# gc00/simgrid

Measured on AMD Instinct MI355X. Metric: LMM solve throughput (vars/s), higher is better.
Workload: dtype f64

## Files before the change

### include/lmm/lmm_hip.h

```cpp
#ifndef LMM_HIP_H
#define LMM_HIP_H

#include <stdint.h>

#ifdef __cplusplus
extern "C" {
#endif

#define LMMHIP_OK 0
#define LMMHIP_E_NODEVICE (-1)
#define LMMHIP_E_HIP (-2)
#define LMMHIP_E_ARG (-3)
#define LMMHIP_E_STATE (-4)
#define LMMHIP_E_NOCONVERGE (-5)

#define LMMHIP_KIND_MAXMIN 0
#define LMMHIP_KIND_FAIR_BOTTLENECK 1

typedef struct lmmhip_ctx lmmhip_ctx;

typedef struct lmmhip_stats {
  int64_t rounds;
  int64_t n_var, n_cnst, nnz;
  double device_ms;
  double kernel_ms[8];
  int64_t kernel_launches[8];
} lmmhip_stats;

int lmmhip_ctx_create(int device, lmmhip_ctx** out);
int lmmhip_ctx_destroy(lmmhip_ctx* ctx);

int lmmhip_upload(lmmhip_ctx* ctx, int64_t n_var, int64_t n_cnst, int64_t nnz, const int64_t* var_ptr,
                  const int32_t* cnst_idx, const double* weight, const double* penalty, const double* var_bound,
                  const double* cnst_bound, const uint8_t* cnst_flags);

int lmmhip_upload2(lmmhip_ctx* ctx, int64_t n_var, int64_t n_cnst, int64_t nnz, const int64_t* var_ptr,
                   const int32_t* cnst_idx, const double* weight, const double* penalty, const double* var_bound,
                   const double* cnst_bound, const uint8_t* cnst_flags, const int64_t* csc_order);

int lmmhip_update_vars(lmmhip_ctx* ctx, const double* penalty, const double* var_bound);
int lmmhip_update_cnsts(lmmhip_ctx* ctx, const double* cnst_bound);

int lmmhip_res_apply(lmmhip_ctx* ctx, int64_t n_elem_total, int64_t n_var_total, int64_t n_cnst_total, int64_t ne,
                     const int64_t* e_id, const int32_t* e_cnst, const double* e_weight, const uint8_t* e_flags,
                     int64_t nv, const int32_t* v_id, const int64_t* v_ebase, const int32_t* v_nelem,
                     const double* v_penalty, const double* v_bound, int64_t nc, const int32_t* c_id,
                     const double* c_bound, const uint8_t* c_flags);
int lmmhip_res_flatten(lmmhip_ctx* ctx, int64_t n_list, const int32_t* cnst_list, double precision, int64_t* counts3);
int lmmhip_res_flatten_fair(lmmhip_ctx* ctx, int64_t n_list, const int32_t* cnst_list, int64_t* counts3);
int lmmhip_res_values(lmmhip_ctx* ctx, int64_t n, double* values, uint8_t* reset);
int lmmhip_res_values_pinned(lmmhip_ctx* ctx, int64_t n, const double** values, const uint8_t** reset);
#define LMMHIP_VAL_KEEP 0x7FF4C0FFEE5107E5ull
int lmmhip_res_values_sliced(lmmhip_ctx* ctx, int64_t n, int nslices, const double** values);
int lmmhip_res_values_wait(lmmhip_ctx* ctx, int slice);
int lmmhip_res_refreshes(lmmhip_ctx* ctx, int64_t* n);
int lmmhip_res_cross_refreshes(lmmhip_ctx* ctx, int64_t* n);
int lmmhip_flat_download(lmmhip_ctx* ctx, int64_t* counts3, uint32_t* var_ptr, int32_t* csr_c, double* csr_w,
                         uint32_t* cnst_ptr, int32_t* csc_v, double* csc_w, double* penalty, double* var_bound,
                         double* cnst_bound, uint8_t* cnst_flags);

int lmmhip_set_batch(lmmhip_ctx* ctx, int64_t nsys, const int64_t* var_off, const int64_t* cnst_off);

int lmmhip_solve(lmmhip_ctx* ctx, int kind, double precision);

int lmmhip_get_values(lmmhip_ctx* ctx, double* values_out);
int lmmhip_get_var_rounds(lmmhip_ctx* ctx, int32_t* rounds_out);
int lmmhip_get_saturated(lmmhip_ctx* ctx, uint8_t* saturated_out);
int lmmhip_get_usage(lmmhip_ctx* ctx, double* usage_out);
int lmmhip_usage_device_ptr(lmmhip_ctx* ctx, const double** dptr);
typedef struct lmmhip_cert {
  double max_excess;
  int64_t n_infeasible, n_unbottlenecked;
  int64_t n_judged_cnst, n_judged_var, n_at_bound;
} lmmhip_cert;
#define LMMHIP_WIT_AT_BOUND (-1)
#define LMMHIP_WIT_NONE (-2)
#define LMMHIP_WIT_NOT_JUDGED (-3)
int lmmhip_certificate(lmmhip_ctx* ctx, double precision, lmmhip_cert* out, int32_t* witness);
int lmmhip_get_touched_vars(lmmhip_ctx* ctx, int32_t* ids, int64_t cap, int64_t* n);
int lmmhip_get_touched_cnsts(lmmhip_ctx* ctx, int32_t* ids, int64_t cap, int64_t* n);
int lmmhip_components(lmmhip_ctx* ctx, int32_t* var_label, int32_t* cnst_label, int64_t* ncomp);
int lmmhip_values_device_ptr(lmmhip_ctx* ctx, const double** dptr);

int lmmhip_get_stats(lmmhip_ctx* ctx, lmmhip_stats* out);
int lmmhip_set_profiling(lmmhip_ctx* ctx, int on);
int lmmhip_launch_profile(lmmhip_ctx* ctx, int* slot, int* round, float* ms, int cap);
int lmmhip_round_profile(lmmhip_ctx* ctx, int64_t* alive_vars, int64_t* alive_elems, int cap);
int lmmhip_vote_profile(lmmhip_ctx* ctx, int64_t* reeval_vars, int64_t* reeval_elems, int cap);
int lmmhip_vote_diag_profile(lmmhip_ctx* ctx, int64_t* out8, int cap);

int lmmhip_ctx_set_stream(lmmhip_ctx* ctx, void* hip_stream);
int lmmhip_ctx_use_own_stream(lmmhip_ctx* ctx);

#define LMMHIP_ENGINE_PERSISTENT 0
#define LMMHIP_ENGINE_ROUNDS 1
#define LMMHIP_ENGINE_AUTO 2
#define LMMHIP_ENGINE_FRONTIER 3
int lmmhip_ctx_set_engine(lmmhip_ctx* ctx, int engine);
int lmmhip_engine_fallbacks(lmmhip_ctx* ctx, int64_t* n);
#define LMMHIP_RAN_PERSISTENT 0
#define LMMHIP_RAN_ROUNDS 1
#define LMMHIP_RAN_FRONTIER 2
#define LMMHIP_RAN_BATCH 3
#define LMMHIP_RAN_FB_ROUNDS 4
#define LMMHIP_RAN_FB_BATCH 5
int lmmhip_last_engine(lmmhip_ctx* ctx, int* engine);
int lmmhip_anatomy(lmmhip_ctx* ctx, unsigned long long* out, int64_t cap, int64_t* n, int32_t* rounds4);
int lmmhip_persist_profile(lmmhip_ctx* ctx, int on, int64_t* t, int64_t cap, int64_t* n);
int lmmhip_persist_profile_blocks(lmmhip_ctx* ctx, int64_t* t, int64_t cap, int64_t* nbar, int64_t* nblk);

int lmmhip_fb_shard_owner(lmmhip_ctx* ctx, int64_t n_own, const int32_t* own_cnst, const int64_t* optr,
                          const int32_t* ovar, const double* oweight, const int32_t* cpos, int64_t n_mu,
                          int64_t n_rem);
int lmmhip_fb_shard_begin(lmmhip_ctx* ctx, double precision, int32_t* xnb, double* xmu, int64_t mu_off,
                          double* xrem);
int lmmhip_fb_shard_step(lmmhip_ctx* ctx, int phase);
int lmmhip_fb_shard_pack_mu(lmmhip_ctx* ctx, int32_t* pos, double* mu, int32_t* count);
int lmmhip_fb_shard_poll(lmmhip_ctx* ctx, int* done, int64_t* rounds);
int lmmhip_fb_work(lmmhip_ctx* ctx, int64_t* out3);

#define LMMHIP_MODEL_CPU 0
#define LMMHIP_MODEL_CM02 1
#define LMMHIP_MODEL_L07 2
#define LMMHIP_EV_FINISHED 1
#define LMMHIP_EV_LATENCY_PAID 2
int lmmhip_actions_upload(lmmhip_ctx* ctx, int64_t n, const int32_t* var_index, const double* remains,
                          const double* max_duration, const double* latency, const double* penalty,
                          const double* sharing_penalty, const uint8_t* flags);
int lmmhip_next_event_full(lmmhip_ctx* ctx, int with_latency, double* out);
int lmmhip_update_actions_full(lmmhip_ctx* ctx, int model, double delta, double maxmin_precision,
                               double surf_precision, int64_t* n_events);
int lmmhip_actions_download(lmmhip_ctx* ctx, double* remains, double* max_duration, double* latency, double* penalty,
                            uint8_t* events);

#define LMMHIP_HEAP_UNSET 0
#define LMMHIP_HEAP_LATENCY 1
#define LMMHIP_HEAP_MAX_DURATION 2
#define LMMHIP_HEAP_NORMAL 3
#define LMMHIP_ACT_NOT_STARTED 4
int lmmhip_actions_lazy_upload(lmmhip_ctx* ctx, const double* last_update, const double* last_value,
                               const double* start_time, const double* date, const uint8_t* heap_type);
int lmmhip_actions_lazy_update(lmmhip_ctx* ctx, int model, double now, double maxmin_precision, double surf_precision,
                               int64_t n_modified, const int32_t* modified, int64_t* n_finished);
int lmmhip_next_event_lazy(lmmhip_ctx* ctx, double now, double* out);
int lmmhip_actions_lazy_due(lmmhip_ctx* ctx, int model, double now, double surf_precision, int32_t* ids,
                            uint8_t* events, int64_t cap, int64_t* n_due);
int lmmhip_actions_lazy_download(lmmhip_ctx* ctx, double* last_update, double* last_value, double* date,
                                 uint8_t* heap_type);

#define LMMHIP_ACT_F_VAR_SLOT 1
#define LMMHIP_ACT_F_REMAINS 2
#define LMMHIP_ACT_F_MAX_DURATION 4
#define LMMHIP_ACT_F_LATENCY 8
#define LMMHIP_ACT_F_PENALTY 16
#define LMMHIP_ACT_F_SHARING_PENALTY 32
#define LMMHIP_ACT_F_FLAGS 64
#define LMMHIP_ACT_F_LAST_UPDATE 128
#define LMMHIP_ACT_F_LAST_VALUE 256
#define LMMHIP_ACT_F_START_TIME 512
#define LMMHIP_ACT_F_DATE 1024
#define LMMHIP_ACT_F_HEAP_TYPE 2048
int lmmhip_actions_bind(lmmhip_ctx* ctx, int64_t n, const int32_t* var_slot);
int lmmhip_actions_patch(lmmhip_ctx* ctx, int64_t k, const int32_t* idx, int fields, const int32_t* var_slot,
                         const double* remains, const double* max_duration, const double* latency,
                         const double* penalty, const double* sharing_penalty, const uint8_t* flags,
                         const double* last_update, const double* last_value, const double* start_time,
                         const double* date, const uint8_t* heap_type);
int lmmhip_actions_lazy_update_solved(lmmhip_ctx* ctx, int model, double now, double maxmin_precision,
                                      double surf_precision, int64_t n_extra, const int32_t* extra,
                                      int64_t* n_modified, int64_t* n_finished);
int lmmhip_actions_events(lmmhip_ctx* ctx, int32_t* ids, uint8_t* events, int64_t cap, int64_t* n);
int lmmhip_actions_var_index(lmmhip_ctx* ctx, int32_t* out);

int lmmhip_device_count(void);

const char* lmmhip_last_error(void);

const char* lmmhip_build_id(void);

#ifdef __cplusplus
}
#endif
// ... 3 lines not shown
```

### simgrid_amd/csrc/lmm_ctx.hpp

```cpp
#pragma once
#include <hip/hip_runtime.h>

#include <cstdlib>

#include <algorithm>
#include <string>
#include <utility>
#include <vector>

#include "../../include/lmm/lmm_hip.h"
#include "lmm_dev.hpp"
#include "lmm_chunk.hpp"
#include "lmm_round_mode.hpp"

using namespace lmmdev;

inline thread_local std::string g_err;

inline int fail(int code, const std::string& msg) {
  g_err = msg;
  return code;
}

#define HIPCHK(expr)                                                                                    \
// ... 3 lines not shown
      return fail(LMMHIP_E_HIP, std::string(#expr " -> ") + hipGetErrorString(e_) + " @" + __FILE__ + \
                                    ":" + std::to_string(__LINE__));                                    \
  } while (0)

inline int env_int(const char* name, int dflt) {
  const char* v = std::getenv(name);
  return v && *v ? std::atoi(v) : dflt;
}

struct DevFree {
  hipError_t operator()(void* p) const { return hipFree(p); }
};
struct PinFree {
  hipError_t operator()(void* p) const { return hipHostFree(p); }
};
struct EventFree {
  hipError_t operator()(hipEvent_t e) const { return hipEventDestroy(e); }
};
struct StreamFree {
  hipError_t operator()(hipStream_t s) const { return hipStreamDestroy(s); }
};
template <class H, class Free> struct Owned {
  H p{};
  Owned() = default;
  Owned(Owned&& o) noexcept : p(std::exchange(o.p, H{})) {}
  Owned& operator=(Owned&& o) noexcept {
    if (this != &o) {
      (void)reset();
      p = std::exchange(o.p, H{});
    }
    return *this;
  }
  ~Owned() { (void)reset(); }
  hipError_t reset() { return p ? Free{}(std::exchange(p, H{})) : hipSuccess; }
};
template <class T> using DevPtr = Owned<T*, DevFree>;
template <class T> using PinPtr = Owned<T*, PinFree>;
using Event = Owned<hipEvent_t, EventFree>;
using Stream = Owned<hipStream_t, StreamFree>;

struct Scr : DevPtr<void> {
  size_t bytes = 0;
  Scr() = default;
  Scr(Scr&& o) noexcept : DevPtr<void>(std::move(o)), bytes(std::exchange(o.bytes, 0)) {}
  Scr& operator=(Scr&& o) noexcept {
    DevPtr<void>::operator=(std::move(o));
    bytes = std::exchange(o.bytes, 0);
    return *this;
  }
};

struct Arena {
  std::vector<void*> v;
  Arena() = default;
  Arena(const Arena&) = delete;
  Arena& operator=(const Arena&) = delete;
  ~Arena() { clear(); }
  void clear() {
    for (void* p : v)
      (void)hipFree(p);
    v.clear();
  }
  template <class T> int alloc(T** out, int64_t n, const T* src = nullptr, hipStream_t stream = nullptr) {
    void* p = nullptr;
    HIPCHK(hipMalloc(&p, size_t(n > 0 ? n : 1) * sizeof(T)));
    v.push_back(p);
    *out = static_cast<T*>(p);
    if (src && n > 0)
      HIPCHK(hipMemcpyAsync(p, src, size_t(n) * sizeof(T), hipMemcpyHostToDevice, stream));
    return 0;
  }
};

struct FlatBufs {
  uint32_t *vp, *cp, *chb;
  int32_t *csr_c, *csc_v, *cvar0, *chc, *cch;
  double *csr_w, *csc_w, *pen, *vb, *cb;
  uint8_t* cf;
};

struct RoundEngine {
  Scr crec[3], rdq[2], rqst, useg, ucnt;
  Scr cmpbits;
};
using VoteKernel = void (*)(Dev, int);
using SatKernel = void (*)(Dev, int, int);
using UpdKernel = void (*)(Dev, int, double);
struct RoundPlan {
  VoteMode mode;
  VoteKernel vote_bitmap = nullptr, vote_scan = nullptr;
  int64_t vote_bits_rows = 0;
  SatKernel saturate = nullptr;
  int sat_waves = 4;
  bool upd_quad = false;
  UpdKernel update = nullptr;
  int g_init_c = 1, g_c = 1;
  int g_upd = 1;
  int cap_sat = 0, sat_max = 0;
  int cmp_every = 48, cmp_pct = 75, cl_every = 8;
  ChunkPolicy chunk;
  int64_t tail_rows = 0, tail_cnst = 0;
};
int solve_maxmin(lmmhip_ctx* c, double prec);

struct FrontierEngine {
  Scr c2s, slot, minfl, qa, qb, qn, md, pvb, key;
  bool map_ok = false;
  int maxdeg = 0;
};
struct FrontierPlan {
  int nblk = 1, nblk_sat = 1;
  int bigch = 1, bigw = 1;
  bool big = false;
  int g_big = 1;
  bool long_rows = false;
  int spb = 1;
  int sat_b = 256;
  int upd_spec = 0;
  ChunkPolicy chunk;
};
int solve_maxmin_frontier(lmmhip_ctx* c, double prec);

int solve_maxmin_persist(lmmhip_ctx* c, double prec);
void persist_ctx_ref(int device, int delta);
constexpr unsigned kPersistProfCap = 1 << 16;

constexpr size_t kBatchLdsMax = 64 * 1024;
bool batch_fits(const lmmhip_ctx* c);
int solve_maxmin_batch(lmmhip_ctx* c, double prec);
int batch_rounds_to_ctl(lmmhip_ctx* c, int grid);
int engine_of(const lmmhip_ctx* c);

struct FairEngine {
  FbFields f{};
  int64_t fbd_cap = 0;
  Scr longl, k0, k1, v0, v1, tmp, perm, cscvp, mu;
  bool perm_ok = false;
  int64_t round = 0;
  double prec = 0;
  uint32_t longmin = 0;
  int nlb = 128;
  int32_t* shard_xnb = nullptr;
  FbOwner owner{};
  bool owner_ready = false;
  int64_t owner_nmu = 0;
  Arena owner_allocs;
};
int solve_fair(lmmhip_ctx* c, double prec);
bool fb_batch_fits(const lmmhip_ctx* c);
int solve_fair_batch(lmmhip_ctx* c, double prec);

struct lmmhip_ctx {
  int device = 0;
  Stream own_stream;
  std::vector<Stream> retired_streams;
  hipStream_t stream = nullptr;
  Dev d{};
  Arena allocs;
  PinPtr<int32_t> h_ctl;
  Event ev_poll[2];
  std::vector<Event> ev_slice;
  bool uploaded = false;
  bool profiling = false;
  int group = 8;
  int n_cu = 256;
  Event ev0, ev1;
  std::vector<Event> pool;
  size_t pool_used = 0;
  std::vector<int> launch_slot, launch_round;
  std::vector<float> launch_ms;
  lmmhip_stats stats{};
  int last_kind = LMMHIP_KIND_MAXMIN;
  int ran_engine = -1;
  int last_engine = -1;
  double last_prec = 1e-5;
  bool solved = false;
  DevPtr<int32_t> vstat;
  DevPtr<unsigned long long> anat;
  int engine = LMMHIP_ENGINE_AUTO;
  int sat_waves = 1;
  bool vote_diag = std::getenv("LMMHIP_VOTE_DIAG") != nullptr;
  DevPtr<unsigned> pbar;
// ... 133 lines not shown
```

### simgrid_amd/csrc/lmm_dev.hpp

```cpp
#pragma once

#include <hip/hip_runtime.h>

#include <cfloat>
#include <climits>
#include <cstdint>
#include <type_traits>

namespace lmmdev {

constexpr int kBlock = 256;
constexpr int kWave = 64;
constexpr int kMaxBlocks = 2048;
constexpr int kRowsPerThread = 8;
constexpr int kCompactRows = kBlock * kRowsPerThread;
constexpr unsigned kDeadKey = 0xFFFFu;
constexpr unsigned kSatKey = 0xFFFEu;
__host__ __device__ constexpr bool key_dead(unsigned k) { return k >= kSatKey; }

enum : int {
  CTL_DONE = 0,
  CTL_ROUNDS = 1,
  CTL_ANY0 = 2,
  CTL_NROWS = 4,
  CTL_NELEM = 7,
  CTL_NREADY = 11,
  CTL_RDQ0 = 12,
  CTL_NCL0 = 14,
  CTL_LASTR = 16,
  CTL_PALIVE0 = 17,
  CTL_ERR = 19,
  CTL_RESEVAL = 20,
  CTL_BUF = 21,
  CTL_CB = 22,
  CTL_CMPGO = 23,
  CTL_FBW = 24,
  CTL_WORDS = 32
};
constexpr int kFbwSlots = 64;
constexpr int CTL_FBW_AT = CTL_WORDS;
constexpr int CTL_ALLOC = CTL_WORDS + 2 * 3 * kFbwSlots;

struct alignas(64) CstRec {
  unsigned long long drem, duse, dcnt;
  int64_t pad;
  double rem, use;
  double ratio;
  double bound;
};
static_assert(sizeof(CstRec) == 64, "CstRec must be one 64-B line");

__device__ __forceinline__ int dec_scale(double m) {
  if (!(m > 0) || !(m < __builtin_huge_val()))
    return 0;
  int s = 61 - __builtin_amdgcn_frexp_exp(m);
  return s < -1000 ? -1000 : (s > 1000 ? 1000 : s);
}
__device__ __forceinline__ unsigned long long dec_q(double d, int s) {
  return (unsigned long long)__double2ll_rn(__builtin_amdgcn_ldexp(d, s));
}
__device__ __forceinline__ double dec_val(unsigned long long q, int s) {
  return __builtin_amdgcn_ldexp(double((long long)q), -s);
}
constexpr int32_t kCexpFat = 1 << 24;
constexpr int32_t kCexpDead = 1 << 25;
__host__ __device__ __forceinline__ int32_t cexp_pack(int srem, int suse, bool fat, bool dead) {
  return int32_t((uint32_t(srem) & 0xFFFu) | ((uint32_t(suse) & 0xFFFu) << 12)) | (fat ? kCexpFat : 0) |
         (dead ? kCexpDead : 0);
}
__device__ __forceinline__ int cexp_rem(int32_t e) { return int32_t(uint32_t(e) << 20) >> 20; }
__device__ __forceinline__ int cexp_use(int32_t e) { return int32_t(uint32_t(e) << 8) >> 20; }

template <class T> __device__ __forceinline__ T ld_rlx(const T* p) {
  return __hip_atomic_load(const_cast<T*>(p), __ATOMIC_RELAXED, __HIP_MEMORY_SCOPE_AGENT);
}
template <class T> __device__ __forceinline__ void st_rlx(T* p, T v) {
  __hip_atomic_store(p, v, __ATOMIC_RELAXED, __HIP_MEMORY_SCOPE_AGENT);
}

union RowRecs {
  uint2* r8;
  uint4* r16;
};

struct Dev {
  int32_t nV, nC;
  int64_t nnz;
  const uint32_t* var_ptr;
  const int32_t* csr_c;
  const double* csr_w;
  const uint32_t* cnst_ptr;
  const int32_t* csc_v;
  const double* csc_w;
  double* csc_u;
  double* csc_p;
  unsigned long long* csc_row;
  const double* pen;
  const double* vbound;
  const double* cbound;
  const uint8_t* cflags;
  uint8_t* cdup;
  double* x;
  unsigned long long* anat;
  int32_t* vstate;
  int32_t anat_r[4];
  double* ratio;
  uint16_t* key;
  double* rem;
  double* use;
  CstRec* cst;
  int32_t* cexp;
  int32_t* nvote;
  uint8_t* ctouch;
  uint16_t* chg;
  int32_t* ready;
  int32_t* bready;
  uint64_t* chgbits;
  int32_t* balive;
  int32_t* clist[2];
// ... 44 lines not shown
  int32_t* vperm;
  int32_t* csc_vp;
  double* mu_p;
  int32_t* hprog;
};

struct FrDev : Dev, FrFields {};
struct FbDev : Dev, FbFields {};
static_assert(std::is_trivially_copyable<FrDev>::value && std::is_trivially_copyable<FbDev>::value,
              "the views are kernel arguments");

__device__ __forceinline__ int rvar(int32_t cv) { return cv & 0x7FFFFFFF; }
__device__ __forceinline__ bool rbounded(int32_t cv) { return cv < 0; }

struct ResDev {
  int32_t* e_cnst;
  double* e_w;
  uint8_t* e_fl;
  int64_t* v_ebase;
  int32_t* v_n;
  double* v_pen;
  double* v_bound;
  double* c_bound;
  uint8_t* c_fl;
};

struct FbOwner {
  int32_t nc;
  int32_t nch;
  int64_t mu_off;
  const int32_t* oc;
  const uint32_t* optr;
  const int32_t* ovar;
  const double* ow;
  const int32_t* och_o;
  const uint32_t* och_b;
  const int32_t* cpos;
  double* fbd;
  double* xmu;
  double* xrem;
};

struct ActDev {
  int64_t n;
  int32_t* vidx;
  double* remains;
  double* max_duration;
  double* latency;
  double* penalty;
  double* share_pen;
  uint8_t* flags;
  uint8_t* events;
  unsigned long long* umin;
  int32_t* nev;
  double* last_update;
  double* last_value;
  double* start_time;
  double* date;
  uint8_t* htype;
  int32_t* due;
  int32_t* ndue;
  int32_t* err;
};

enum : int { BIND_NONE = 0, BIND_DENSE = 1, BIND_RESIDENT = 2 };
struct ActBind {
  int mode;
  int64_t nv;
  const int64_t* vm;
  const int64_t* dv;
};

constexpr int kFbChunk = 1024;
constexpr int kDiagSlot = kMaxBlocks - 4;
constexpr unsigned kPBlkCap = 1024;

constexpr int kStatRounds = 4096;
constexpr int32_t kUnvoted = -1;
constexpr unsigned long long kValKeep = 0x7FF4C0FFEE5107E5ull;
constexpr int32_t kRetired = -2;

__device__ __forceinline__ double dinf() { return __builtin_huge_val(); }

#ifndef LMM_KEY_MANT
#define LMM_KEY_MANT 7
#endif
__device__ __forceinline__ uint16_t ratio_key(double r) {
  float f = __double2float_rd(r);
  return uint16_t(__float_as_uint(f) >> (23 - LMM_KEY_MANT));
}

constexpr uint32_t kDead32 = 0xFFFFFFFFu;
__device__ __forceinline__ uint32_t ratio_key32(double r) { return __float_as_uint(__double2float_rd(r)); }

template <int W> __device__ __forceinline__ double grp_min(double v) {
#pragma unroll
  for (int o = W / 2; o > 0; o >>= 1)
    v = fmin(v, __shfl_xor(v, o, W));
  return v;
}
template <int W> __device__ __forceinline__ unsigned grp_umin(unsigned v) {
#pragma unroll
  for (int o = W / 2; o > 0; o >>= 1)
    v = min(v, (unsigned)__shfl_xor((int)v, o, W));
  return v;
}
template <int W> __device__ __forceinline__ int grp_imin(int v) {
#pragma unroll
  for (int o = W / 2; o > 0; o >>= 1)
    v = min(v, __shfl_xor(v, o, W));
  return v;
}
template <int W> __device__ __forceinline__ int grp_isum(int v) {
#pragma unroll
  for (int o = W / 2; o > 0; o >>= 1)
    v += __shfl_xor(v, o, W);
  return v;
}
__device__ __forceinline__ double wave_sum(double v) {
#pragma unroll
  for (int o = 32; o > 0; o >>= 1)
    v += __shfl_xor(v, o, kWave);
  return v;
}
__device__ __forceinline__ double wave_max(double v) {
#pragma unroll
  for (int o = 32; o > 0; o >>= 1)
    v = fmax(v, __shfl_xor(v, o, kWave));
  return v;
}
__device__ __forceinline__ double wave_min(double v) {
#pragma unroll
  for (int o = 32; o > 0; o >>= 1)
    v = fmin(v, __shfl_xor(v, o, kWave));
  return v;
}

__device__ __forceinline__ int wave_append(bool pred, int32_t* counter) {
  const unsigned long long m = __ballot(pred);
  if (!m)
    return -1;
  const int lane = threadIdx.x & (kWave - 1);
  const int leader = __ffsll((long long)m) - 1;
  int base = 0;
  if (lane == leader)
    base = atomicAdd(counter, __popcll(m));
  base = __shfl(base, leader, kWave);
  return pred ? base + __popcll(m & ((1ull << lane) - 1)) : -1;
}

__device__ __forceinline__ int block_append(bool pred, int32_t* counter) {
  __shared__ int wcnt[kBlock / kWave];
  __shared__ int bbase;
  const int lane = threadIdx.x & (kWave - 1), w = threadIdx.x / kWave;
  const unsigned long long m = __ballot(pred);
  if (lane == 0)
    wcnt[w] = __popcll(m);
  __syncthreads();
  if (threadIdx.x == 0) {
    int tot = 0;
    for (int i = 0; i < kBlock / kWave; i++) {
      const int c = wcnt[i];
      wcnt[i] = tot;
      tot += c;
    }
    bbase = tot ? atomicAdd(counter, tot) : 0;
  }
  __syncthreads();
  const int pos = bbase + wcnt[w] + __popcll(m & ((1ull << lane) - 1));
  __syncthreads();
  return pred ? pos : -1;
}
// ... 114 lines not shown
```

### simgrid_amd/csrc/lmm_frontier_kernels.hpp

```cpp
#pragma once
#include "lmm_maxmin_kernels.hpp"

namespace lmmdev {

constexpr int kFB = 256;
constexpr uint32_t kNoVoter = 0xFFFFFFFFu;
constexpr int kFrBigCh = 16;
constexpr int kFrBigWaves = 16;
constexpr int kFVS = 4;

__global__ void __launch_bounds__(kBlock) fr_c2s(FrDev s, int2* cs, int32_t* maxdeg) {
  const int lane = threadIdx.x & (kWave - 1);
  int md = 0;
  for (int64_t c = (int64_t(blockIdx.x) * kBlock + threadIdx.x) / kWave; c < s.nC;
       c += int64_t(gridDim.x) * (kBlock / kWave)) {
    const uint32_t b = s.cnst_ptr[c], e = s.cnst_ptr[c + 1];
    md = max(md, int(e - b));
    const bool dup = s.cdup[c] != 0;
    bool sorted_col = true;
    if (dup) {
      bool desc = false;
      for (uint32_t j = b + 1 + lane; j < e; j += kWave)
        desc |= s.csc_v[j - 1] > s.csc_v[j];
      sorted_col = __ballot(desc) == 0;
    }
    for (uint32_t j = b + lane; j < e; j += kWave) {
      const int32_t v = s.csc_v[j];
      const unsigned long long row = s.csc_row[j];
      int occ = 0;
      if (dup && sorted_col)
        for (uint32_t i = j; i > b && s.csc_v[i - 1] == v; i--)
          occ++;
      else if (dup)
        for (uint32_t i = b; i < j; i++)
          occ += s.csc_v[i] == v;
      for (uint32_t k = uint32_t(row); k < uint32_t(row >> 32); k++)
        if (s.csr_c[k] == int32_t(c) && occ-- == 0) {
          cs[k] = make_int2(int32_t(c), int32_t(j));
          break;
        }
    }
  }
  md = -grp_imin<kWave>(-md);
  if (lane == 0 && md)
    atomicMax(maxdeg, md);
}

__global__ void __launch_bounds__(kBlock) fr_init_vars(FrDev s) {
  const int64_t stride = int64_t(gridDim.x) * kBlock;
  for (int64_t v = int64_t(blockIdx.x) * kBlock + threadIdx.x; v < s.nV; v += stride) {
    s.x[v] = 0.0;
    s.vstate[v] = 0;
    s.rtgt[0][v] = kUnvoted;
    s.pvb[v] = make_double2(s.vbound[v], s.pen[v]);
  }
  uint4* vs4 = reinterpret_cast<uint4*>(s.vslot);
  const uint4 none = make_uint4(kNoVoter, kNoVoter, kNoVoter, kNoVoter);
  for (int64_t j = int64_t(blockIdx.x) * kBlock + threadIdx.x; j < s.nnz / 4; j += stride)
    vs4[j] = none;
  for (int64_t j = (s.nnz & ~int64_t(3)) + int64_t(blockIdx.x) * kBlock + threadIdx.x; j < s.nnz; j += stride)
    s.vslot[j] = kNoVoter;
  for (int64_t c = int64_t(blockIdx.x) * kBlock + threadIdx.x; c < s.nC; c += stride)
    s.minfl[c] = kNoVoter;
}

__device__ __forceinline__ void fr_diag(const Dev& s, int round, int k, bool pred) {
  if (!s.vstat || round >= kStatRounds)
    return;
  const unsigned long long m = __ballot(pred);
  if (m && (threadIdx.x & (kWave - 1)) == __ffsll((long long)m) - 1)
    atomicAdd(s.vstat + 2 * (int64_t(round) * kMaxBlocks + kDiagSlot) + k, __popcll(m));
}
__device__ __forceinline__ void fr_diag_n(const Dev& s, int round, int k, int n) {
  if (!s.vstat || round >= kStatRounds)
    return;
  n = grp_isum<kWave>(n);
  if ((threadIdx.x & (kWave - 1)) == 0 && n)
    atomicAdd(s.vstat + 2 * (int64_t(round) * kMaxBlocks + kDiagSlot) + k, n);
}

enum : int { FR_STAY = 0, FR_MOVE = 1, FR_BOUND = 2, FR_DROP = 3 };

__device__ __forceinline__ uint32_t row_floor32(uint32_t sk, uint32_t mk, double vb, double p) {
  uint32_t fl = sk;
  if (vb > 0)
    fl = min(fl, ratio_key32(vb * p));
  return fl <= mk ? 0u : fl;
}

template <int R, bool kMinfl = true, bool kEarly = true>
__device__ __forceinline__ int fr_revote(const FrDev& s, int v, int t, uint32_t b, uint32_t e, int round, Anat an) {
  const uint32_t* __restrict__ key = s.key32;
  const double2 bp = s.pvb[v];
  const double vb = bp.x, p = bp.y;
  int32_t cc[R];
  uint32_t sl[R];
#pragma unroll
  for (int i = 0; i < R; i++) {
    const int2 x = b + i < e ? s.csr_cs[b + i] : make_int2(-1, 0);
    cc[i] = x.x;
    sl[i] = uint32_t(x.y);
  }
  if (an.on()) {
    int sc = 0;
#pragma unroll
    for (int i = 0; i < R; i++)
      sc += cc[i] + int(sl[i]);
    an.level(1, vb + p + double(sc));
  }
  uint32_t kk[R], mf[R];
#pragma unroll
  for (int i = 0; i < R; i++) {
    kk[i] = cc[i] >= 0 ? key[cc[i]] : kDead32;
    mf[i] = kMinfl && kEarly && cc[i] >= 0 ? s.minfl[cc[i]] : 0u;
  }
  if (an.on()) {
    uint32_t sk0 = 0;
#pragma unroll
    for (int i = 0; i < R; i++)
      sk0 += kk[i] + mf[i];
    an.level(2, sk0);
  }
  uint32_t mk = kDead32;
#pragma unroll
  for (int i = 0; i < R; i++)
    mk = min(mk, kk[i]);
#pragma unroll 4
  for (uint32_t j = b + R; j < e; j++)
    mk = min(mk, key[s.csr_cs[j].x]);
  if (mk == kDead32) {
    s.vstate[v] = round + 1;
    return FR_DROP;
  }
  int nmin = 0, mult_old = 0, newt = INT_MAX;
  uint32_t kt = kDead32;
#pragma unroll
  for (int i = 0; i < R; i++) {
    nmin += kk[i] == mk;
    if (cc[i] == t) {
      mult_old++;
      kt = kk[i];
    }
    if (kk[i] == mk)
      newt = min(newt, cc[i]);
  }
#pragma unroll 4
  for (uint32_t j = b + R; j < e; j++) {
    const int32_t c = s.csr_cs[j].x;
    const uint32_t k = key[c];
    nmin += k == mk;
    if (c == t) {
      mult_old++;
      kt = k;
    }
    if (k == mk)
      newt = min(newt, c);
  }
  double minr = dinf();
  if (nmin > 1 || vb > 0) {
    newt = INT_MAX;
    double rr[R];
#pragma unroll
    for (int i = 0; i < R; i++)
      rr[i] = kk[i] == mk ? s.cst[cc[i]].ratio : dinf();
#pragma unroll
    for (int i = 0; i < R; i++)
      if (kk[i] == mk && (rr[i] < minr || (rr[i] == minr && cc[i] < newt))) {
        minr = rr[i];
        newt = cc[i];
      }
    for (uint32_t j = b + R; j < e; j++) {
      const int32_t c = s.csr_cs[j].x;
      if (key[c] == mk) {
        const double r = s.cst[c].ratio;
        if (r < minr || (r == minr && c < newt)) {
          minr = r;
          newt = c;
        }
      }
    }
  }
  an.level(3, minr + double(newt + nmin));
  if (vb > 0 && vb * p < minr) {
    s.vstate[v] = round + 1;
    s.x[v] = vb;
    if (t >= 0 && kt != kDead32)
      atomicAdd(&s.nvote[t], mult_old);
    for (uint32_t j = b; j < e; j++)
      push_decrement(s, j, vb, p);
    return FR_BOUND;
  }
  uint32_t sk = kDead32;
  int mult_new = 0;
  uint32_t slot = 0xFFFFFFFFu;
  uint32_t mfn = kNoVoter;
#pragma unroll
  for (int i = 0; i < R; i++) {
    if (cc[i] != newt) {
      sk = min(sk, kk[i]);
    } else {
      mult_new++;
      slot = min(slot, sl[i]);
      mfn = kEarly ? mf[i] : kNoVoter;
    }
  }
  for (uint32_t j = b + R; j < e; j++) {
    const int2 x = s.csr_cs[j];
    if (x.x != newt) {
      sk = min(sk, key[x.x]);
    } else {
      mult_new++;
      slot = min(slot, uint32_t(x.y));
      mfn = kNoVoter;
    }
  }
  const uint32_t fl = min(row_floor32(sk, mk, vb, p), kNoVoter - 1u);
  if (kMinfl && !kEarly)
    mfn = s.minfl[newt];
  s.vslot[slot] = fl;
  if (kMinfl && fl < mfn)
    atomicMin(&s.minfl[newt], fl);
  if (newt == t) {
    an.level(4, 0u);
    return FR_STAY;
  }
  if (t >= 0 && kt != kDead32)
    atomicAdd(&s.nvote[t], mult_old);
  atomicSub(&s.nvote[newt], mult_new);
  s.rtgt[0][v] = newt;
  an.level(4, 0u);
  return FR_MOVE;
}

__global__ void __launch_bounds__(kBlock) fr_vote_all(FrDev s) {
  for (int64_t v = int64_t(blockIdx.x) * kBlock + threadIdx.x; v < s.nV; v += int64_t(gridDim.x) * kBlock)
    fr_revote<8, false>(s, int(v), kUnvoted, s.var_ptr[v], s.var_ptr[v + 1], 0, Anat());
}

__global__ void __launch_bounds__(kBlock) fr_minfl_all(FrDev s) {
  const int lane = threadIdx.x & (kWave - 1), gl = lane & 15;
  const int64_t wave = (int64_t(blockIdx.x) * kBlock + threadIdx.x) / kWave;
  const int64_t nwaves = int64_t(gridDim.x) * (kBlock / kWave);
  for (int64_t c = wave * 4 + lane / 16; c < s.nC; c += nwaves * 4) {
    const uint32_t b = s.cnst_ptr[c], e = s.cnst_ptr[c + 1];
    uint32_t m = kNoVoter;
    for (uint32_t j = b + gl; j < e; j += 64) {
      uint32_t f[4];
#pragma unroll
      for (int k = 0; k < 4; k++)
        f[k] = j + 16 * k < e ? s.vslot[j + 16 * k] : kNoVoter;
#pragma unroll
      for (int k = 0; k < 4; k++)
        m = min(m, f[k]);
    }
    m = grp_umin<16>(m);
    if (gl == 0)
      s.minfl[c] = m;
  }
}

template <int R>
__device__ __forceinline__ void fr_vote_blk(const FrDev& s, int round, int spb, int vb, Anat an, Anat ar) {
  const int64_t nseg = (int64_t(s.nC) + kFB - 1) / kFB;
  int n[kFVS], pre[kFVS + 1];
  uint32_t seg[kFVS];
  pre[0] = 0;
#pragma unroll
  for (int k = 0; k < kFVS; k++) {
    const int64_t sg = int64_t(vb) * spb + k;
    n[k] = k < spb && sg < nseg ? s.fq_n[sg] : 0;
    seg[k] = k < spb && sg < nseg ? s.cnst_ptr[sg * kFB] : 0u;
    pre[k + 1] = pre[k] + n[k];
  }
  an.level(0, pre[kFVS] + int(seg[0]));
  an.count(0, unsigned(pre[kFVS]));
  for (int i = threadIdx.x; i < pre[kFVS]; i += kFB) {
    int k = 0;
#pragma unroll
    for (int q = 1; q < kFVS; q++)
      k += i >= pre[q];
    const uint32_t at = seg[k] + uint32_t(i - pre[k]);
    ar.restart();
    an.count(1);
    const unsigned long long a = s.fq_a[at], rw = s.fq_b[at];
    ar.level(0, a + rw);
    const int o = fr_revote<R, true, false>(s, int(uint32_t(a)), int(uint32_t(a >> 32)), uint32_t(rw),
                                             uint32_t(rw >> 32), round, ar);
    if (s.vstat) {
      fr_diag(s, round, 6, true);
      fr_diag(s, round, 4, o == FR_MOVE);
      fr_diag(s, round, 7, o == FR_BOUND);
    }
  }
}

template <int R = 8> __global__ void __launch_bounds__(kFB) fr_vote(FrDev s, int round, int spb) {
  AnatWave aw, awr;
  const Anat an = aw.open(s, round, ANAT_VOTE), ar = awr.open(s, round, ANAT_VOTE);
  const unsigned long long t_in = an.restart();
// ... 566 lines not shown
```

### simgrid_amd/csrc/lmm_hip.hip

```cpp
#include <cstring>

#include "lmm_ctx.hpp"
#include "lmm_common_kernels.hpp"
#include "lmm_cc_kernels.hpp"
#include "lmm_scan.hpp"

void free_owner(lmmhip_ctx* c) {
  c->fair.owner_allocs.clear();
  c->fair.owner = FbOwner{};
  c->fair.owner_ready = false;
}

static void free_all(lmmhip_ctx* c) {
  c->allocs.clear();
  free_owner(c);
  c->d = Dev{};
  c->uploaded = false;
  c->fair.f = FbFields{};
  c->fair.fbd_cap = 0;
  c->fair.shard_xnb = nullptr;
  c->res_flat = false;
}

const char* lmmhip_last_error(void) { return g_err.c_str(); }
// ... 577 lines not shown
  HIPCHK(hipStreamSynchronize(c->stream));
  c->stream = static_cast<hipStream_t>(stream);
  return 0;
}

int lmmhip_ctx_use_own_stream(lmmhip_ctx* c) {
  if (!c)
    return fail(LMMHIP_E_ARG, "null context");
  HIPCHK(hipSetDevice(c->device));
  HIPCHK(hipStreamSynchronize(c->stream));
  c->stream = c->own_stream.p;
  return 0;
}

int lmmhip_persist_profile(lmmhip_ctx* c, int on, int64_t* t, int64_t cap, int64_t* n) {
  if (!c)
    return fail(LMMHIP_E_ARG, "null context");
  c->persist_prof = on != 0;
  if (n)
    *n = 0;
  if (!t || !c->ptime.p)
    return 0;
  HIPCHK(hipSetDevice(c->device));
  std::vector<long long> h(2 * size_t(kPersistProfCap));
  HIPCHK(hipMemcpyAsync(h.data(), c->ptime.p, h.size() * sizeof(long long), hipMemcpyDeviceToHost, c->stream));
  HIPCHK(hipStreamSynchronize(c->stream));
  int64_t m = 0;
  while (m < int64_t(kPersistProfCap) && h[2 * size_t(m) + 1] != 0)
    m++;
  for (int64_t i = 0; i < m && 2 * i + 1 < cap; i++) {
    t[2 * i] = h[2 * size_t(i)];
    t[2 * i + 1] = h[2 * size_t(i) + 1];
  }
  if (n)
    *n = m;
  return 0;
}

int lmmhip_persist_profile_blocks(lmmhip_ctx* c, int64_t* t, int64_t cap, int64_t* nbar, int64_t* nblk) {
  if (!c || !c->ptime.p || !c->persist_grid)
    return fail(LMMHIP_E_STATE, "no profiled persistent solve");
  HIPCHK(hipSetDevice(c->device));
  const size_t n = 2 * size_t(kPBlkCap) * size_t(c->persist_grid);
  std::vector<long long> h(n);
  HIPCHK(hipMemcpyAsync(h.data(), c->ptime.p + 2 * size_t(kPersistProfCap), n * sizeof(long long),
                        hipMemcpyDeviceToHost, c->stream));
  HIPCHK(hipStreamSynchronize(c->stream));
  for (size_t i = 0; i < n && int64_t(i) < cap; i++)
    t[i] = h[i];
  *nbar = kPBlkCap;
  *nblk = c->persist_grid;
  return 0;
}

int lmmhip_anatomy(lmmhip_ctx* c, unsigned long long* out, int64_t cap, int64_t* n, int32_t* rounds4) {
  if (!c || !n)
    return fail(LMMHIP_E_ARG, "null argument");
  const int64_t words = int64_t(kAnatSlots) * kAnatKernels * kAnatWaves * kAnatFields;
  *n = 0;
  if (!LMM_ANAT)
    return fail(LMMHIP_E_STATE, "not an anatomy build (make EXTRA_HIPFLAGS=-DLMM_ANAT=1)");
  if (!c->anat.p || !c->solved)
    return fail(LMMHIP_E_STATE, "no solve recorded an anatomy (set LMMHIP_ANAT_ROUNDS)");
  *n = words;
  if (rounds4)
    for (int k = 0; k < kAnatSlots; k++)
      rounds4[k] = c->d.anat_r[k];
  if (out) {
    if (cap < words)
      return fail(LMMHIP_E_ARG, "anatomy: cap too small");
    HIPCHK(hipSetDevice(c->device));
    HIPCHK(hipMemcpy(out, c->anat.p, size_t(words) * sizeof(unsigned long long), hipMemcpyDeviceToHost));
  }
  return 0;
}

int lmmhip_engine_fallbacks(lmmhip_ctx* c, int64_t* n) {
  if (!c || !n)
    return fail(LMMHIP_E_ARG, "null argument");
  *n = c->persist_fallbacks;
  return 0;
}

int lmmhip_ctx_set_engine(lmmhip_ctx* c, int engine) {
  if (!c)
    return fail(LMMHIP_E_ARG, "null context");
  if (engine != LMMHIP_ENGINE_PERSISTENT && engine != LMMHIP_ENGINE_ROUNDS && engine != LMMHIP_ENGINE_AUTO &&
      engine != LMMHIP_ENGINE_FRONTIER)
    return fail(LMMHIP_E_ARG, "unknown maxmin engine");
  c->engine = engine;
  return 0;
}

int lmmhip_launch_profile(lmmhip_ctx* c, int* slot, int* round, float* ms, int cap) {
  if (!c)
    return fail(LMMHIP_E_ARG, "null context");
  int n = int(c->launch_ms.size());
  for (int i = 0; i < n && i < cap; i++) {
    slot[i] = c->launch_slot[size_t(i)];
    round[i] = c->launch_round[size_t(i)];
    ms[i] = c->launch_ms[size_t(i)];
  }
  return n;
}

int lmmhip_round_profile(lmmhip_ctx* c, int64_t* alive_vars, int64_t* alive_elems, int cap) {
  if (!c || !c->uploaded)
    return fail(LMMHIP_E_STATE, "no system uploaded");
  const int64_t nV = c->d.nV;
  std::vector<int32_t> fr(size_t(nV > 0 ? nV : 1));
  std::vector<uint32_t> vp(size_t(nV) + 1);
  HIPCHK(hipSetDevice(c->device));
  if (nV) {
    const int32_t* src = c->last_kind == LMMHIP_KIND_MAXMIN ? c->d.vstate : c->fair.f.fixr;
    HIPCHK(hipMemcpyAsync(fr.data(), src, sizeof(int32_t) * nV, hipMemcpyDeviceToHost, c->stream));
    HIPCHK(hipMemcpyAsync(vp.data(), c->d.var_ptr, sizeof(uint32_t) * (nV + 1), hipMemcpyDeviceToHost, c->stream));
  }
  HIPCHK(hipStreamSynchronize(c->stream));
  if (c->last_kind == LMMHIP_KIND_MAXMIN)
    for (auto& f : fr)
      f -= 1;
  const int R = int(c->stats.rounds);
  std::vector<int64_t> dv(size_t(R) + 2, 0), de(size_t(R) + 2, 0);
  for (int64_t v = 0; v < nV; v++) {
    int f = fr[size_t(v)];
    if (f < 0)
      continue;
    if (f > R)
      f = R;
    dv[size_t(f)] += 1;
    de[size_t(f)] += vp[size_t(v) + 1] - vp[size_t(v)];
  }
  int64_t av = 0, ae = 0;
  for (int r = R; r >= 0; r--) {
    av += dv[size_t(r)];
    ae += de[size_t(r)];
    if (r < cap) {
      alive_vars[r] = av;
      alive_elems[r] = ae;
    }
  }
  return R;
}

int lmmhip_vote_profile(lmmhip_ctx* c, int64_t* rows, int64_t* elems, int cap) {
  if (!c || !c->vstat.p)
    return fail(LMMHIP_E_STATE, "no profiled maxmin solve");
  const int R = int(std::min<int64_t>(c->stats.rounds, kStatRounds));
  std::vector<int32_t> h(size_t(2) * kStatRounds * kMaxBlocks);
  HIPCHK(hipSetDevice(c->device));
  HIPCHK(hipMemcpy(h.data(), c->vstat.p, sizeof(int32_t) * h.size(), hipMemcpyDeviceToHost));
  for (int r = 0; r < R && r < cap; r++) {
    int64_t a = 0, b = 0;
    for (int k = 0; k < kDiagSlot; k++) {
      a += h[2 * (size_t(r) * kMaxBlocks + k)];
      b += h[2 * (size_t(r) * kMaxBlocks + k) + 1];
    }
    rows[r] = a;
    elems[r] = b;
  }
  return R;
}

int lmmhip_vote_diag_profile(lmmhip_ctx* c, int64_t* out8, int cap) {
  if (!c || !c->vstat.p)
    return fail(LMMHIP_E_STATE, "no profiled maxmin solve");
// ... 254 lines not shown
```

### simgrid_amd/csrc/lmm_hip_maxmin.hip

```cpp
#include <cstring>

#include <array>
#include <map>
#include <mutex>
#include <thread>
#include <utility>

#include "lmm_ctx.hpp"
#include "lmm_maxmin_kernels.hpp"
#include "lmm_persist_kernels.hpp"
#include "lmm_frontier_kernels.hpp"
#include "lmm_batch_kernels.hpp"

constexpr int64_t kAutoPersistVars = 1 << 18;
constexpr int64_t kAutoPersistMaxVars = 1 << 14;

namespace {
std::mutex g_persist_mu;
std::map<int, Event>& g_persist_last = *new std::map<int, Event>;
std::map<int, int> g_persist_users;
}

void persist_ctx_ref(int device, int delta) {
  std::lock_guard<std::mutex> lk(g_persist_mu);
  int& n = g_persist_users[device];
  n += delta;
  if (n <= 0) {
    g_persist_users.erase(device);
    g_persist_last.erase(device);
  }
}


template <class Rounds, class ChunkEnd, class InTail>
static int run_chunks(lmmhip_ctx* c, const Dev& d, const ChunkPolicy& p, Rounds&& round_launches, ChunkEnd&& chunk_end,
                      InTail&& in_tail) {
  const int64_t max_rounds = int64_t(d.nV) + 2;
  CtlPoll poll;
  if (int rc = poll.init(c))
    return rc;
  int chunk = p.first;
  for (int64_t r = 0;;) {
    bool stop = false;
    const int n = round_hint_chunk(r, chunk, p.hint, &stop);
    for (int k = 0; k < n; k++, r++)
      if (int rc = round_launches(r))
        return rc;
    if (int rc = chunk_end(r))
      return rc;
    const int32_t* h = nullptr;
    if (int rc = poll.step(d, r, stop, &h))
      return rc;
    if (h && h[CTL_DONE])
      break;
    const bool tail = in_tail(h);
    if (h && h[CTL_ROUNDS] > max_rounds)
      return fail(LMMHIP_E_NOCONVERGE, "maxmin round guard tripped");
    chunk = chunk_grow(chunk, p, tail);
  }
  return poll_ctl(c);
}

struct VoteKernels {
  VoteKernel bitmap, scan;
};
template <int... I> constexpr std::array<VoteKernels, sizeof...(I)> lane_votes(std::integer_sequence<int, I...>) {
  return {{{mm_vote_lane<VoteForm::Bitmap, I>, mm_vote_lane<VoteForm::Scan, I>}...}};
}
constexpr auto kVoteTable = lane_votes(std::make_integer_sequence<int, kVoteModes>{});
constexpr VoteKernel kVoteLong[3] = {mm_vote<16>, mm_vote<32>, mm_vote<64>};
constexpr SatKernel kSatTable[2][3] = {{mm_saturate<1>, mm_saturate<2>, mm_saturate<4>},
                                       {mm_saturate_q<1>, mm_saturate_q<2>, mm_saturate_q<4>}};
template <int... I> constexpr std::array<UpdKernel, sizeof...(I)> updates(std::integer_sequence<int, I...>) {
  return {{mm_update<I>...}};
}
constexpr auto kUpdTable = updates(std::make_integer_sequence<int, kUpdModes>{});

static RoundPlan round_plan(const lmmhip_ctx* c, const Dev& d) {
  RoundPlan P;
  RoundKnobs k;
  k.crec = env_int("LMMHIP_CREC", 1);
  k.rdq = env_int("LMMHIP_RDQ", 1);
  k.satkey = env_int("LMMHIP_SATKEY", 1);
  k.cmp_rows = env_int("LMMHIP_CMP_ROWS", 1);
  k.upd_quad = env_int("LMMHIP_UPD_QUAD", 1);
  k.upd_blocks = env_int("LMMHIP_UPD_BLOCKS", 0);
  k.updq_blocks = env_int("LMMHIP_UPDQ_BLOCKS", updq_blocks_default(c->n_cu));
  const RoundMode m = resolve_round_mode(c->group, d.nC, k, RoundLimits{kBlock, kUSeg, kMaxBlocks});
  P.mode = m.vote;
  P.upd_quad = m.upd_quad;
  P.g_upd = m.g_upd;
  P.cap_sat = env_int("LMMHIP_SAT_BLOCKS", 5 * c->n_cu);
  const bool short_rows = c->group == 4 || c->group == 8;
  const VoteKernels vk = short_rows ? kVoteTable[P.mode.index()]
                                    : VoteKernels{nullptr, kVoteLong[c->group == 16 ? 0 : c->group == 32 ? 1 : 2]};
  const bool bits = int64_t(d.nC) <= int64_t(kBitWords) * 64 && env_int("LMMHIP_VOTE_BITS", 1) != 0;
  P.vote_bitmap = bits ? vk.bitmap : nullptr;
  P.vote_scan = vk.scan;
  P.vote_bits_rows = env_int("LMMHIP_VOTE_BITS_ROWS", 0);
  const int sat_k = env_int("LMMHIP_SAT_WAVES", c->sat_waves);
  P.sat_waves = sat_k == 1 || sat_k == 2 ? sat_k : 4;
  P.saturate = kSatTable[P.mode.rdq()][P.sat_waves == 4 ? 2 : P.sat_waves - 1];
  P.sat_max = env_int("LMMHIP_SAT_GRID_MAX", kMaxBlocks);
  P.update = kUpdTable[m.upd().index()];
  P.g_init_c = grid_for(d.nC, kBlock / kWave);
  P.g_c = grid_for(d.nC, kBlock);
  P.cmp_every = env_int("LMMHIP_COMPACT_EVERY", 48);
  P.cmp_pct = env_int("LMMHIP_COMPACT_PCT", 75);
  P.cl_every = env_int("LMMHIP_CLIST_EVERY", 8);
  P.chunk.hint = env_int("LMMHIP_ROUND_HINT", 1) ? c->hint_rounds_mm : 0;
  P.chunk.first = 2;
  P.chunk.max = std::max(2, env_int("LMMHIP_CHUNK_MAX", P.chunk.hint > 0 ? 64 : 32));
  P.tail_rows = env_int("LMMHIP_CHUNK_TAIL_ROWS",
                        int(int64_t(d.nV) * std::max(0, env_int("LMMHIP_CHUNK_TAIL_PCT", 5)) / 100));
  P.tail_cnst = env_int("LMMHIP_CHUNK_TAIL_CNST", 0);
  P.chunk.tail = std::max(1, env_int("LMMHIP_CHUNK_TAIL", 4));
  return P;
}

static int round_buffers(lmmhip_ctx* c, Dev& d, const RoundPlan& P, uint8_t** cmpbits) {
  for (int k = 0; k < 3 && P.mode.rec(); k++)
    if (int rc = P.mode.rec16() ? scratch(c, c->rounds.crec[k], int64_t(d.nV) + 1, &d.crec[k].r16)
                                : scratch(c, c->rounds.crec[k], int64_t(d.nV) + 1, &d.crec[k].r8))
      return rc;
  if (P.mode.rec16())
    if (int rc = scratch(c, c->rounds.cmpbits, (int64_t(d.nV) + kCompactRows - 1) / kCompactRows * kBlock, cmpbits))
      return rc;
  if (P.mode.rdq()) {
    const int64_t n = std::max<int64_t>(d.nC, 1);
    if (int rc = scratch(c, c->rounds.rdq[0], n, &d.rdq[0]) | scratch(c, c->rounds.rdq[1], n, &d.rdq[1]) |
                 scratch(c, c->rounds.rqst, n, &d.rqst) | scratch(c, c->rounds.useg, int64_t(P.g_upd) * kUSeg, &d.useg) |
                 scratch(c, c->rounds.ucnt, kMaxBlocks, &d.ucnt))
      return rc;
    HIPCHK(hipMemsetAsync(d.rqst, 0xFF, size_t(n) * sizeof(int32_t), c->stream));
    HIPCHK(hipMemsetAsync(d.ucnt, 0, size_t(kMaxBlocks) * sizeof(int32_t), c->stream));
  }
  return 0;
}

static int launch_vote(lmmhip_ctx* c, const Dev& d, const RoundPlan& P, int64_t r, int64_t nrows) {
  const bool bitmap = P.vote_bitmap && nrows >= P.vote_bits_rows;
  if (bitmap && c->profiling && c->vote_diag) {
    LAUNCH(7, r + 1000000, (mm_vote_lane<VoteForm::Bitmap, kVoteArrays, 2>), c->n_cu, kVBlock, d, int(r));
    LAUNCH(7, r, (mm_vote_lane<VoteForm::Bitmap, kVoteArrays, 1>), c->n_cu, kVBlock, d, int(r));
    LAUNCH(7, r, mm_vote_diagcount, grid_for((int64_t(d.nC) + 63) / 64, kBlock), kBlock, d, int(r));
  }
  LAUNCH(2, r, bitmap ? P.vote_bitmap : P.vote_scan, bitmap ? c->n_cu : grid_for(nrows, kBlock), bitmap ? kVBlock : kBlock,
         d, int(r));
  return 0;
}

int solve_maxmin(lmmhip_ctx* c, double prec) {
  c->ran_engine = LMMHIP_RAN_ROUNDS;
  Dev d = c->d;
  const RoundPlan P = round_plan(c, d);
  uint8_t* cmpbits = nullptr;
  if (int rc = round_buffers(c, d, P, &cmpbits))
    return rc;
  LAUNCH(0, -1, mm_init_cnsts, P.g_init_c, kBlock, d, static_cast<uint32_t*>(nullptr), prec);
  LAUNCH(1, -1, mm_init_vars, grid_for(d.nV, kBlock), kBlock, d, int(P.mode.rec16()));
  LAUNCH(1, -1, mm_clist, std::min(P.g_c, 2 * c->n_cu), kBlock, d, 1);
  HIPCHK(hipMemsetAsync(d.chgbits, 0, sizeof(uint64_t) * ((d.nC + 127) / 128 * 2 + 2), c->stream));
  int64_t last_compact = 0, last_clist = 0, nrows = d.nV, ncl = d.nC;
  auto round_launches = [&](int64_t r) -> int {
    if (int rc = launch_vote(c, d, P, r, nrows))
      return rc;
    const int gL = grid_for(ncl, kBlock);
    if (!P.mode.rdq())
      LAUNCH(3, r, mm_ready, gL, kBlock, d);
    const int64_t gS = std::max<int64_t>(1, std::min<int64_t>((P.sat_waves * ncl + kBlock - 1) / kBlock, P.sat_max));
    LAUNCH(4, r, P.saturate, int(P.cap_sat > 0 && gS > P.cap_sat ? P.cap_sat : gS), kBlock, d, int(r),
           P.mode.rdq() ? P.g_upd : gL);
    LAUNCH(5, r, P.update, P.g_upd, kBlock, d, int(r), prec);
    return 0;
  };
  auto chunk_end = [&](int64_t r) -> int {
    LAUNCH(6, r, mm_done, 1, kBlock, d, P.g_upd);
    const int gL = grid_for(ncl, kBlock);
    bool cl = false, cm = false;
    if (r - last_clist >= P.cl_every && ncl > 4096) {
      LAUNCH(6, r, mm_clist, std::min(gL, 2 * c->n_cu), kBlock, d, 0);
      last_clist = r;
      cl = true;
    }
    if (r - last_compact >= P.cmp_every && nrows > 4096) {
      const int nblk = int((nrows + kCompactRows - 1) / kCompactRows);
      switch (P.mode.form) {
        case RowForm::Rec16:
          LAUNCH(6, r, cmp_count_rows, nblk, kBlock, d, cmpbits);
          LAUNCH(6, r, cmp_scan<true>, 1, 1024, d, nblk, P.cmp_pct);
          LAUNCH(6, r, cmp_write_rows, nblk, kBlock, d, cmpbits);
          break;
        case RowForm::Arrays:
        case RowForm::Rec8:
          LAUNCH(6, r, cmp_count, nblk, kBlock, d);
          LAUNCH(6, r, cmp_scan<false>, 1, 1024, d, nblk, P.cmp_pct);
          LAUNCH(6, r, cmp_write, nblk, kBlock, d);
          break;
      }
      last_compact = r;
      cm = true;
    }
    if (cl || cm)
      LAUNCH(6, r, mm_flip, 1, 1, d, int(cl), int(cm));
    return 0;
  };
  auto in_tail = [&](const int32_t* h) {
    if (h) {
      ncl = h[CTL_NCL0 + h[CTL_CB]];
      nrows = h[CTL_NROWS + h[CTL_BUF]];
    }
    return nrows <= P.tail_rows || ncl <= P.tail_cnst;
  };
  if (int rc = run_chunks(c, d, P.chunk, round_launches, chunk_end, in_tail))
    return rc;
  c->hint_rounds_mm = int64_t(c->h_ctl.p[CTL_LASTR]) + 1;
  return 0;
}

static FrontierPlan frontier_plan(const lmmhip_ctx* c, const Dev& d) {
  FrontierPlan P;
  P.nblk = int(std::max<int64_t>(1, (int64_t(d.nC) + kFB - 1) / kFB));
  P.nblk_sat = int(std::max<int64_t>(1, (int64_t(d.nC) + kFS - 1) / kFS));
  P.bigch = std::max(1, env_int("LMMHIP_FR_BIGCH", kFrBigCh));
  P.big = c->frontier.maxdeg > P.bigch * kWave;
  P.bigw = std::max(1, env_int("LMMHIP_FR_BIGW", kFrBigWaves));
  P.g_big = std::min(kMaxBlocks, 4 * c->n_cu);
  P.long_rows = c->group > 8 && env_int("LMMHIP_FR_R16", 1) != 0;
  P.spb = int(std::max<int64_t>(1, std::min<int64_t>(kFVS, int64_t(P.nblk) / (2 * int64_t(c->n_cu)))));
  const int sat_b0 = int64_t(P.nblk_sat) >= 2 * int64_t(c->n_cu) ? kFS : 256;
  P.sat_b = env_int("LMMHIP_FR_SATB", sat_b0) == 256 ? 256 : kFS;
  P.upd_spec = env_int("LMMHIP_FR_UPDSPEC", P.sat_b == 256 ? 1 : 0);
  const int chunk_max = std::max(2, env_int("LMMHIP_CHUNK_MAX", 8));
  P.chunk.hint = env_int("LMMHIP_ROUND_HINT", 1) ? c->hint_rounds_fr : 0;
  P.chunk.max = P.chunk.hint > 0 ? std::max(chunk_max, env_int("LMMHIP_HINT_CHUNK_MAX", 32)) : chunk_max;
  P.chunk.first = 2;
  if (P.chunk.hint > 0)
    P.chunk.first = std::max(2, std::min(P.chunk.max, env_int("LMMHIP_HINT_CHUNK0", P.chunk.max)));
  return P;
}

int solve_maxmin_frontier(lmmhip_ctx* c, double prec) {
  c->ran_engine = LMMHIP_RAN_FRONTIER;
  FrDev d{c->d, FrFields{}};
  if (!c->vote_diag)
    d.vstat = nullptr;
  const int64_t nnz = std::max<int64_t>(d.nnz, 1);
  const int64_t nblk = std::max<int64_t>(1, (int64_t(d.nC) + kFB - 1) / kFB);
  int2* cs = nullptr;
  int32_t* md = nullptr;
  int rc = scratch(c, c->frontier.c2s, nnz, &cs);
  rc = rc ? rc : scratch(c, c->frontier.pvb, std::max<int64_t>(d.nV, 1), &d.pvb);
  rc = rc ? rc : scratch(c, c->frontier.slot, nnz, &d.vslot);
  rc = rc ? rc : scratch(c, c->frontier.minfl, std::max<int64_t>(d.nC, 1), &d.minfl);
  rc = rc ? rc : scratch(c, c->frontier.key, std::max<int64_t>(d.nC, 1), &d.key32);
  rc = rc ? rc : scratch(c, c->frontier.qa, nnz, &d.fq_a);
  rc = rc ? rc : scratch(c, c->frontier.qb, nnz, &d.fq_b);
  rc = rc ? rc : scratch(c, c->frontier.qn, nblk + 1, &d.fq_n);
  rc = rc ? rc : scratch(c, c->frontier.md, 1, &md);
  if (rc)
    return rc;
  d.csr_cs = cs;
  if (!c->frontier.map_ok) {
    HIPCHK(hipMemsetAsync(md, 0, sizeof(int32_t), c->stream));
    if (d.nnz > 0) {
      hipLaunchKernelGGL(fr_c2s, dim3(grid_for(d.nC, kBlock / kWave)), dim3(kBlock), 0, c->stream, d, cs, md);
      HIPCHK(hipGetLastError());
    }
    HIPCHK(hipMemcpyAsync(&c->frontier.maxdeg, md, sizeof(int32_t), hipMemcpyDeviceToHost, c->stream));
    HIPCHK(hipStreamSynchronize(c->stream));
    c->frontier.map_ok = true;
  }
  const FrontierPlan P = frontier_plan(c, d);
  LAUNCH(0, -1, mm_init_cnsts, grid_for(d.nC, kBlock / kWave), kBlock, d, d.key32, prec);
  LAUNCH(1, -1, fr_init_vars, grid_for(std::max<int64_t>(std::max<int64_t>(d.nV, d.nC), d.nnz / 4), kBlock), kBlock, d);
  auto round_launches = [&](int64_t r) -> int {
    if (r == 0) {
      LAUNCH(2, r, fr_vote_all, grid_for(d.nV, kBlock), kBlock, d);
      LAUNCH(2, r, fr_minfl_all, grid_for(d.nC, kBlock / 16), kBlock, d);
    } else if (P.long_rows) {
      LAUNCH(2, r, fr_vote<16>, (P.nblk + P.spb - 1) / P.spb, kFB, d, int(r), P.spb);
    } else {
      LAUNCH(2, r, fr_vote<8>, (P.nblk + P.spb - 1) / P.spb, kFB, d, int(r), P.spb);
    }
    if (P.sat_b == 256)
      LAUNCH(4, r, fr_sat<256>, P.nblk, 256, d, int(r), P.bigch);
    else
      LAUNCH(4, r, fr_sat<kFS>, P.nblk_sat, kFS, d, int(r), P.bigch);
    if (P.big)
      LAUNCH(4, r, fr_sat_big, P.g_big, kBlock, d, int(r), P.bigw);
    LAUNCH(5, r, fr_update, P.nblk, kFB, d, int(r), prec, P.upd_spec);
    return 0;
  };
  if (int rc = run_chunks(c, d, P.chunk, round_launches, [](int64_t) { return 0; }, [](const int32_t*) { return false; }))
    return rc;
  c->hint_rounds_fr = int64_t(c->h_ctl.p[CTL_ROUNDS]) + 1;
  return 0;
}

int engine_of(const lmmhip_ctx* c) {
  const char* e = std::getenv("LMMHIP_ENGINE");
  int eng = c->engine;
  if (e && std::strcmp(e, "rounds") == 0)
    eng = LMMHIP_ENGINE_ROUNDS;
  if (e && std::strcmp(e, "persistent") == 0)
    eng = LMMHIP_ENGINE_PERSISTENT;
  if (e && std::strcmp(e, "frontier") == 0)
    eng = LMMHIP_ENGINE_FRONTIER;
  if (c->profiling)
    return eng == LMMHIP_ENGINE_FRONTIER ? LMMHIP_ENGINE_FRONTIER : LMMHIP_ENGINE_ROUNDS;
  if (eng != LMMHIP_ENGINE_AUTO)
    return eng;
  if (int64_t(c->d.nV) <= kAutoPersistMaxVars)
    return LMMHIP_ENGINE_PERSISTENT;
  return int64_t(c->d.nV) <= kAutoPersistVars ? LMMHIP_ENGINE_FRONTIER : LMMHIP_ENGINE_ROUNDS;
}


static int solve_maxmin_persist_once(lmmhip_ctx* c, double prec, bool* closed) {
  Dev d = c->d;
  d.vstat = nullptr;
  const bool bits = int64_t(d.nC) <= int64_t(kPBitWords) * 64;
  const void* kern = bits ? reinterpret_cast<const void*>(&mm_persist<true, 8>)
                          : reinterpret_cast<const void*>(&mm_persist<false, 8>);
  if (!c->pbar.p)
    HIPCHK(hipMalloc(reinterpret_cast<void**>(&c->pbar.p), BAR_WORDS * sizeof(unsigned)));
  int per_cu = 0;
  HIPCHK(hipOccupancyMaxActiveBlocksPerMultiprocessor(&per_cu, kern, kPB, 0));
  if (per_cu < 1)
    return fail(LMMHIP_E_HIP, "persistent maxmin kernel: not one workgroup per CU (occupancy query)");
  const int grid = c->n_cu;
  c->persist_grid = grid;
  const int max_rounds = int(std::min<int64_t>(int64_t(d.nV) + 2, INT32_MAX - 1));
  const int cmp_every = env_int("LMMHIP_COMPACT_EVERY", 16);
  unsigned* barw = c->pbar.p;
  long long* pt = nullptr;
  unsigned pt_cap = 0;
  if (c->persist_prof) {
    pt_cap = kPersistProfCap;
    const size_t bytes = sizeof(long long) * (2 * size_t(pt_cap) + 2 * size_t(kPBlkCap) * size_t(grid));
    if (!c->ptime.p)
      HIPCHK(hipMalloc(reinterpret_cast<void**>(&c->ptime.p), bytes));
    HIPCHK(hipMemsetAsync(c->ptime.p, 0, bytes, c->stream));
    pt = c->ptime.p;
  }
  int sysf = env_int("LMMHIP_PERSIST_SYSFENCE", 0);
  long long rdv_ticks = 100000LL * env_int("LMMHIP_PERSIST_RDV_MS", 20);
  int32_t* hflag = c->d_rdv;
  void* args[] = {&d, &barw, &prec, const_cast<int*>(&max_rounds), const_cast<int*>(&cmp_every), &pt, &pt_cap, &sysf,
                  &rdv_ticks, &hflag};
  {
    std::lock_guard<std::mutex> lk(g_persist_mu);
    Event& last = g_persist_last[c->device];
    if (last.p && hipStreamWaitEvent(c->stream, last.p, 0) != hipSuccess) {
      (void)hipGetLastError();
      (void)last.reset();
    }
// ... 182 lines not shown
```

### simgrid_amd/csrc/lmm_maxmin_kernels.hpp

```cpp
#pragma once
#include <type_traits>

#include "lmm_dev.hpp"
#include "lmm_round_mode.hpp"

namespace lmmdev {


constexpr int kInitG = 16;
__device__ __forceinline__ int init_cnsts_waves(const Dev& s, uint32_t* key32, double prec, int64_t wave,
                                                int64_t nwaves) {
  const int lane = threadIdx.x & (kWave - 1), gl = lane & (kInitG - 1);
  constexpr int kGpw = kWave / kInitG;
  int alive_cnt = 0;
  for (int64_t c = wave * kGpw + lane / kInitG; c < s.nC; c += nwaves * kGpw) {
    const uint32_t b = s.cnst_ptr[c], e = s.cnst_ptr[c + 1];
    const bool fat = s.cflags[c] & 1;
    double acc = 0.0;
    for (uint32_t j0 = b + gl; j0 < e; j0 += 4 * kInitG) {
      double u[4];
#pragma unroll
      for (int k = 0; k < 4; k++)
        u[k] = j0 + k * kInitG < e ? s.csc_u[j0 + k * kInitG] : 0.0;
#pragma unroll
      for (int k = 0; k < 4; k++)
        acc = fat ? fmax(acc, u[k]) : acc + u[k];
    }
#pragma unroll
    for (int o = kInitG / 2; o > 0; o >>= 1) {
      const double y = __shfl_xor(acc, o, kInitG);
      acc = fat ? fmax(acc, y) : acc + y;
    }
    if (gl == 0) {
      const double bound = s.cbound[c];
      const bool part = bound > bound * prec;
      const double usage = part ? acc : 0.0;
      const bool alive = part && usage > 0;
      const double r = bound / usage;
      CstRec rec;
      rec.drem = rec.duse = rec.dcnt = 0;
      rec.pad = 0;
      s.ctouch[c] = 0;
      rec.rem = bound;
      rec.use = usage;
      rec.ratio = alive ? r : dinf();
      rec.bound = bound;
      s.cst[c] = rec;
      s.cexp[c] = cexp_pack(alive ? dec_scale(bound) : 0, alive ? dec_scale(usage) : 0, fat, !alive);
      s.nvote[c] = int32_t(e - b);
      s.chg[c] = uint16_t(0xFFFF);
      s.key[c] = alive ? ratio_key(r) : uint16_t(kDeadKey);
      if (key32)
        key32[c] = alive ? ratio_key32(r) : kDead32;
      alive_cnt += alive;
    }
  }
  return alive_cnt;
}

__global__ void __launch_bounds__(kBlock) mm_init_cnsts(Dev s, uint32_t* key32, double prec) {
  const int64_t wave = (int64_t(blockIdx.x) * kBlock + threadIdx.x) / kWave;
  init_cnsts_waves(s, key32, prec, wave, int64_t(gridDim.x) * (kBlock / kWave));
}

template <RowForm F>
__device__ __forceinline__ void init_vars_range(const Dev& s, int64_t t, int64_t nthreads) {
  for (int64_t v = t; v < s.nV; v += nthreads) {
    s.x[v] = 0.0;
    s.vstate[v] = 0;
    s.rtgt[0][v] = kUnvoted;
    const int32_t cv = int32_t(v) | (s.vbound[v] > 0 ? int32_t(0x80000000u) : 0);
    const_cast<int32_t*>(s.cvar[0])[v] = cv;
    if (F == RowForm::Rec16)
      s.crec[0].r16[v] = make_uint4(uint32_t(cv), s.var_ptr[v], s.var_ptr[v + 1], 0u);
    else if (F == RowForm::Rec8 && s.crec[0].r8)
      s.crec[0].r8[v] = make_uint2(uint32_t(cv), s.var_ptr[v]);
  }
}

__global__ void __launch_bounds__(kBlock) mm_init_vars(Dev s, int rec16) {
  const int64_t t = int64_t(blockIdx.x) * kBlock + threadIdx.x, nthreads = int64_t(gridDim.x) * kBlock;
  if (rec16)
    init_vars_range<RowForm::Rec16>(s, t, nthreads);
  else
    init_vars_range<RowForm::Rec8>(s, t, nthreads);
  if (blockIdx.x == 0 && threadIdx.x == 0) {
    s.ctl[CTL_NROWS + 0] = s.nV;
    s.ctl[CTL_NELEM + 0] = int32_t(s.nnz);
    if (!rec16 && s.crec[0].r8)
      s.crec[0].r8[s.nV] = make_uint2(0u, s.var_ptr[s.nV]);
  }
}

constexpr int kUSeg = 1024;
__device__ __forceinline__ void rdq_push(const Dev& s, int32_t c, int qround) {
  if (atomicExch(&s.rqst[c], qround) != qround) {
    const int q = qround & 1;
    s.rdq[q][atomicAdd(&s.ctl[CTL_RDQ0 + q], 1)] = c;
  }
}
constexpr int kRqCap = 2048;
struct RdqLds {
  int n, base;
  int32_t buf[kRqCap];
};
__device__ __forceinline__ void rdq_push_lds(const Dev& s, int32_t c, int qround, RdqLds* L) {
  if (c >= 0 && atomicExch(&s.rqst[c], qround) != qround) {
    const int pos = atomicAdd(&L->n, 1);
    if (pos < kRqCap) {
      L->buf[pos] = c;
    } else {
      const int q = qround & 1;
      s.rdq[q][atomicAdd(&s.ctl[CTL_RDQ0 + q], 1)] = c;
    }
  }
}
__device__ __forceinline__ void rdq_flush_lds(const Dev& s, int qround, RdqLds* L) {
  __syncthreads();
  const int n = L->n < kRqCap ? L->n : kRqCap;
  const int q = qround & 1;
  if (threadIdx.x == 0)
    L->base = n ? atomicAdd(&s.ctl[CTL_RDQ0 + q], n) : 0;
  __syncthreads();
  for (int i = threadIdx.x; i < n; i += blockDim.x)
    s.rdq[q][L->base + i] = L->buf[i];
}

__device__ __forceinline__ unsigned row_floor(unsigned sk, unsigned mk, double vb, double p) {
  unsigned fl = sk;
  if (vb > 0)
    fl = min(fl, (unsigned)ratio_key(vb * p));
  return fl <= mk ? 0u : fl;
}

__device__ __forceinline__ unsigned long long fat_bits(double u) { return (unsigned long long)__double_as_longlong(u); }

__device__ __forceinline__ void push_decrement(const Dev& s, uint32_t j, double xv, double p) {
  const int32_t c = s.csr_c[j];
  const int32_t ce = s.cexp[c];
  if (ce & kCexpDead)
    return;
  unsigned long long* r = &s.cst[c].drem;
  s.ctouch[c] = 1;
  atomicAdd(&r[2], 1ull);
  const double w = s.csr_w[j];
  if (!(ce & kCexpFat)) {
    atomicAdd(&r[0], dec_q(w * xv, cexp_rem(ce)));
    atomicAdd(&r[1], dec_q(w / p, cexp_use(ce)));
  } else {
    atomicMax(&r[1], fat_bits(w / p));
  }
}

template <int G> __global__ void __launch_bounds__(kBlock) mm_vote(Dev s, int round) {
  if (s.ctl[CTL_DONE])
    return;
  const int buf = s.ctl[CTL_BUF];
  __shared__ int st_rows, st_elems;
  if (s.vstat && threadIdx.x == 0)
    st_rows = st_elems = 0;
  if (s.vstat)
    __syncthreads();
  const int64_t nrows = s.ctl[CTL_NROWS + buf];
  const int32_t* __restrict__ cvar = s.cvar[buf];
  const uint32_t* __restrict__ crow = s.crow[buf];
  const int32_t* __restrict__ ccol = s.ccol[buf];
  const uint16_t* __restrict__ key = s.key;
  const int lane = threadIdx.x & (kWave - 1);
  const int g = lane & (G - 1);
  constexpr int kGpw = kWave / G;
  const int64_t wave = (int64_t(blockIdx.x) * kBlock + threadIdx.x) / kWave;
  const int64_t nwaves = int64_t(gridDim.x) * (kBlock / kWave);
  int32_t* __restrict__ rtgt = s.rtgt[buf];
  const uint16_t prev = uint16_t(round - 1);
  for (int64_t base = wave * kWave; base < nrows; base += nwaves * kWave) {
    const int64_t lrow = base + lane;
    const int lt = lrow < nrows ? rtgt[lrow] : kRetired;
    const bool lneed = lt == kUnvoted || (lt >= 0 && s.chg[lt] == prev &&
                                          (key_dead(key[lt]) || !(key[lt] < s.skey[buf][lrow])));
    unsigned long long mask = __ballot(lneed);
    while (mask) {
      unsigned long long m = mask;
      for (int i = 0; i < lane / G; i++)
        m &= m - 1;
      const int pos = m ? __ffsll((long long)m) - 1 : -1;
      for (int i = 0; i < kGpw; i++)
        mask &= mask - 1;
      const int src = pos < 0 ? 0 : pos;
      const int t = __shfl(lt, src, kWave);
      const int64_t row = base + src;
      const int v = pos >= 0 ? rvar(cvar[row]) : 0;
      bool need = pos >= 0;
      if (need && s.vstate[v] != 0) {
        if (g == 0)
          rtgt[row] = kRetired;
        need = false;
      }
      uint32_t b = 0, e = 0;
      if (need) {
        b = crow[row];
        e = crow[row + 1];
        if (s.vstat && g == 0) {
          atomicAdd(&st_rows, 1);
          atomicAdd(&st_elems, int(e - b));
        }
      }
      const uint32_t j0 = b + g;
      const bool h0 = j0 < e;
      const int32_t c0 = h0 ? ccol[j0] : -1;
      const unsigned k0 = h0 ? key[c0] : kDeadKey;
      unsigned mk = k0;
      for (uint32_t j = j0 + G; j < e; j += G)
        mk = min(mk, (unsigned)key[ccol[j]]);
      mk = grp_umin<G>(mk);
      int nmin = h0 && k0 == mk;
      for (uint32_t j = j0 + G; j < e; j += G)
        nmin += key[ccol[j]] == mk;
      nmin = grp_isum<G>(nmin);
      const double vb = need ? s.vbound[v] : -1.0;
      const bool live = need && !key_dead(mk);
      double minr = dinf();
      if (live && (nmin > 1 || vb > 0)) {
        if (h0 && k0 == mk)
          minr = s.cst[c0].ratio;
        for (uint32_t j = j0 + G; j < e; j += G) {
          const int32_t c = ccol[j];
          if (key[c] == mk)
            minr = fmin(minr, s.cst[c].ratio);
        }
      }
      minr = grp_min<G>(minr);
      const double p = need ? s.pen[v] : 1.0;
      const bool bounded = live && vb > 0 && vb * p < minr;
      int newt = INT_MAX;
      if (live && !bounded) {
        if (h0 && k0 == mk && (nmin == 1 || s.cst[c0].ratio == minr))
          newt = c0;
        for (uint32_t j = j0 + G; j < e; j += G) {
          const int32_t c = ccol[j];
          if (key[c] == mk && (nmin == 1 || s.cst[c].ratio == minr))
            newt = min(newt, c);
        }
      }
      newt = grp_imin<G>(newt);
      unsigned sk = h0 && c0 != newt ? k0 : kDeadKey;
      for (uint32_t j = j0 + G; j < e; j += G) {
        const int32_t c = ccol[j];
        if (c != newt)
          sk = min(sk, (unsigned)key[c]);
      }
      sk = grp_umin<G>(sk);
      if (live && !bounded && g == 0)
        s.skey[buf][row] = uint16_t(row_floor(sk, mk, vb, p));
      int mult_new = h0 && c0 == newt, mult_old = h0 && c0 == t;
      for (uint32_t j = j0 + G; j < e; j += G) {
        const int32_t c = ccol[j];
        mult_new += c == newt;
        mult_old += c == t;
      }
      mult_new = grp_isum<G>(mult_new);
      mult_old = grp_isum<G>(mult_old);
      if (need && !live) {
        if (g == 0) {
          s.vstate[v] = round + 1;
          rtgt[row] = kRetired;
        }
      } else if (bounded) {
        if (g == 0) {
          s.vstate[v] = round + 1;
          s.x[v] = vb;
          rtgt[row] = kRetired;
          if (t >= 0 && !key_dead(key[t]))
            atomicAdd(&s.nvote[t], mult_old);
        }
        for (uint32_t j = s.var_ptr[v] + g; j < s.var_ptr[v + 1]; j += G)
          push_decrement(s, j, vb, p);
      } else if (live && newt != t && g == 0) {
        if (t >= 0 && !key_dead(key[t]))
          atomicAdd(&s.nvote[t], mult_old);
        atomicSub(&s.nvote[newt], mult_new);
        rtgt[row] = newt;
      }
    }
  }
  if (s.vstat) {
    __syncthreads();
    if (threadIdx.x == 0 && round < kStatRounds && blockIdx.x < kMaxBlocks) {
      s.vstat[2 * (int64_t(round) * kMaxBlocks + blockIdx.x)] = st_rows;
      s.vstat[2 * (int64_t(round) * kMaxBlocks + blockIdx.x) + 1] = st_elems;
    }
  }
}

__global__ void __launch_bounds__(kBlock) mm_clist(Dev s, int from_all) {
  if (!from_all && s.ctl[CTL_DONE])
    return;
  __shared__ int wsum[kBlock / kWave];
  __shared__ int base_sh;
  const int in = from_all ? 0 : s.ctl[CTL_CB], out = from_all ? 0 : in ^ 1;
  const int64_t n = from_all ? s.nC : s.ctl[CTL_NCL0 + in];
  const int64_t per = (n + gridDim.x - 1) / gridDim.x;
  const int64_t lo = int64_t(blockIdx.x) * per, hi = lo + per < n ? lo + per : n;
  const int lane = threadIdx.x & (kWave - 1), w = threadIdx.x / kWave;
  int cnt = 0;
  for (int64_t i = lo + threadIdx.x; i < hi; i += kBlock) {
    const int32_t c = from_all ? int32_t(i) : s.clist[in][i];
    cnt += !key_dead(s.key[c]);
  }
  cnt = grp_isum<kWave>(cnt);
  if (lane == 0)
    wsum[w] = cnt;
  __syncthreads();
  if (threadIdx.x == 0) {
    int t = 0;
    for (int k = 0; k < kBlock / kWave; k++)
      t += wsum[k];
    base_sh = t ? atomicAdd(&s.ctl[CTL_NCL0 + out], t) : 0;
  }
  __syncthreads();
  int pos = base_sh;
  for (int64_t b0 = lo; b0 < hi; b0 += kBlock) {
    const int64_t i = b0 + threadIdx.x;
    int32_t c = -1;
    if (i < hi)
      c = from_all ? int32_t(i) : s.clist[in][i];
    const bool alive = c >= 0 && !key_dead(s.key[c]);
    const unsigned long long m = __ballot(alive);
    __syncthreads();
    if (lane == 0)
      wsum[w] = __popcll(m);
    __syncthreads();
    int off = pos, tot = 0;
    for (int k = 0; k < kBlock / kWave; k++) {
      off += k < w ? wsum[k] : 0;
      tot += wsum[k];
    }
    if (alive)
      s.clist[out][off + __popcll(m & ((1ull << lane) - 1))] = c;
    pos += tot;
  }
}

__global__ void mm_flip(Dev s, int clist, int rows) {
  if (s.ctl[CTL_DONE])
    return;
  if (clist) {
    const int in = s.ctl[CTL_CB];
    s.ctl[CTL_CB] = in ^ 1;
    s.ctl[CTL_NCL0 + in] = 0;
  }
  if (rows && s.ctl[CTL_CMPGO]) {
    const int in = s.ctl[CTL_BUF];
    s.ctl[CTL_BUF] = in == 1 ? 2 : 1;
  }
}

#ifndef LMM_KFILT
#define LMM_KFILT 8
#endif
constexpr int kFilt = LMM_KFILT;

template <int R, int M>
__device__ __forceinline__ void vote_row(const Dev& s, int buf, int round, int64_t row, int* st_rows,
                                         int* st_elems, const uint16_t* __restrict__ key, int* rdq_c = nullptr,
                                         Anat an = Anat()) {
  static_assert(vote_mode_ok(M), "not one of the nine vote modes");
  constexpr VoteMode vm = vote_mode(M);
  an.restart();
  const int32_t* __restrict__ cvar = s.cvar[buf];
  const uint32_t* __restrict__ crow = s.crow[buf];
  const int32_t* __restrict__ ccol = s.ccol[vm.rec16() ? 0 : buf];
  int32_t* __restrict__ rtgt = s.rtgt[buf];
  uint16_t* __restrict__ skey = s.skey[buf];
  const int t = rtgt[row];
  int32_t cv;
  uint32_t b, e;
  if (vm.rec16()) {
    const uint4 r = s.crec[buf].r16[row];
    cv = int32_t(r.x);
    b = r.y;
    e = r.z;
  } else if (vm.rec()) {
    const uint2 r0 = s.crec[buf].r8[row], r1 = s.crec[buf].r8[row + 1];
    cv = int32_t(r0.x);
    b = r0.y;
    e = r1.y;
  } else {
    cv = cvar[row];
    b = crow[row];
    e = crow[row + 1];
  }
  an.level(0, b + e + uint32_t(t) + uint32_t(cv));
  const int v = rvar(cv);
  const int32_t vst = !vm.sat_retire() || t == kUnvoted ? s.vstate[v] : 0;
  const bool bnd = rbounded(cv);
  const double vb = bnd ? s.vbound[v] : -1.0;
  const double p = bnd ? s.pen[v] : 1.0;
  an.level(1, vst);
  if (vst != 0) {
    rtgt[row] = kRetired;
    return;
  }
  if (s.vstat) {
    atomicAdd(st_rows, 1);
    atomicAdd(st_elems, int(e - b));
  }
  int32_t cc[R];
  unsigned kk[R];
#pragma unroll
  for (int i = 0; i < R; i++)
    cc[i] = b + i < e ? ccol[b + i] : -1;
  if (an.on()) {
    int32_t ccs = 0;
#pragma unroll
    for (int i = 0; i < R; i++)
      ccs += cc[i];
    an.level(2, ccs);
  }
#pragma unroll
  for (int i = 0; i < R; i++)
    kk[i] = cc[i] >= 0 ? key[cc[i]] : kDeadKey;
  const unsigned kt = t >= 0 ? key[t] : kDeadKey;
  unsigned mk = kDeadKey;
#pragma unroll
  for (int i = 0; i < R; i++)
    mk = min(mk, kk[i]);
#pragma unroll 4
  for (uint32_t j = b + R; j < e; j++)
    mk = min(mk, (unsigned)key[ccol[j]]);
  an.level(3, mk + kt);
  if (key_dead(mk)) {
    s.vstate[v] = round + 1;
    rtgt[row] = kRetired;
    return;
  }
  int nmin = 0, mult_old = 0, newt = INT_MAX;
#pragma unroll
  for (int i = 0; i < R; i++) {
    nmin += kk[i] == mk;
    mult_old += cc[i] == t;
    if (kk[i] == mk)
      newt = min(newt, cc[i]);
  }
#pragma unroll 4
  for (uint32_t j = b + R; j < e; j++) {
    const int32_t c = ccol[j];
    const unsigned k = key[c];
    nmin += k == mk;
    mult_old += c == t;
    if (k == mk)
      newt = min(newt, c);
  }
  double minr = dinf();
  if (nmin > 1 || vb > 0) {
    newt = INT_MAX;
    constexpr bool kTieLd = vm.tie_loads();
    double rr[kTieLd ? R : 1];
    if (kTieLd) {
#pragma unroll
      for (int i = 0; i < R; i++)
        rr[kTieLd ? i : 0] = kk[i] == mk ? s.cst[cc[i]].ratio : dinf();
    }
#pragma unroll
    for (int i = 0; i < R; i++)
      if (kk[i] == mk) {
        const double r = kTieLd ? rr[kTieLd ? i : 0] : s.cst[cc[i]].ratio;
        if (r < minr || (r == minr && cc[i] < newt)) {
          minr = r;
          newt = cc[i];
        }
      }
    for (uint32_t j = b + R; j < e; j++) {
      const int32_t c = ccol[j];
      if (key[c] == mk) {
        const double r = s.cst[c].ratio;
        if (r < minr || (r == minr && c < newt)) {
          minr = r;
          newt = c;
        }
      }
    }
  }
  an.level(4, minr + double(newt));
  if (vb > 0 && vb * p < minr) {
    s.vstate[v] = round + 1;
    s.x[v] = vb;
    rtgt[row] = kRetired;
    if (t >= 0 && !key_dead(kt))
      atomicAdd(&s.nvote[t], mult_old);
    for (uint32_t j = s.var_ptr[v]; j < s.var_ptr[v + 1]; j++)
      push_decrement(s, j, vb, p);
    return;
  }
  unsigned sk = kDeadKey;
  int mult_new = 0;
#pragma unroll
  for (int i = 0; i < R; i++) {
    if (cc[i] != newt)
      sk = min(sk, kk[i]);
    mult_new += cc[i] == newt;
  }
#pragma unroll 4
  for (uint32_t j = b + R; j < e; j++) {
    const int32_t c = ccol[j];
    const unsigned k = key[c];
    if (c != newt)
      sk = min(sk, k);
    mult_new += c == newt;
  }
  skey[row] = uint16_t(row_floor(sk, mk, vb, p));
  if (newt == t)
    return;
  if (t >= 0 && !key_dead(kt))
    atomicAdd(&s.nvote[t], mult_old);
  if (vm.rdq()) {
    const int old = atomicSub(&s.nvote[newt], mult_new);
    if (old == mult_new) {
      if (rdq_c)
        *rdq_c = newt;
      else
        rdq_push(s, newt, round);
    }
    an.level(5, old);
  } else {
    atomicSub(&s.nvote[newt], mult_new);
  }
  rtgt[row] = newt;
}

constexpr int kQW = 2 * kWave;

__device__ __forceinline__ void vote_wave_range(int64_t lo, int64_t hi, int64_t& wlo, int64_t& whi) {
  const int w = threadIdx.x / kWave, nw = blockDim.x / kWave;
  const int64_t ngr = (hi - lo + kWave - 1) / kWave;
  const int64_t gpw = (ngr + nw - 1) / nw;
  wlo = lo + int64_t(w) * gpw * kWave;
  whi = wlo + gpw * kWave < hi ? wlo + gpw * kWave : hi;
}

template <bool kBits, int R, int F, int kDiag, int M>
__device__ __forceinline__ int vote_waves(const Dev& s, int buf, int round, int64_t lo, int64_t hi,
                                          const uint64_t* bits, int* qw, int* st_rows, int* st_elems,
                                          const uint16_t* __restrict__ key, RdqLds* rql = nullptr, Anat an = Anat(),
                                          Anat ar = Anat()) {
  constexpr VoteMode vm = vote_mode(M);
  const int lane = threadIdx.x & (kWave - 1);
  int64_t wlo, whi;
  vote_wave_range(lo, hi, wlo, whi);
  const int32_t* __restrict__ rtgt = s.rtgt[buf];
  const uint16_t* __restrict__ skey = s.skey[buf];
  const uint16_t prev = uint16_t(round - 1);
  const unsigned long long below = (1ull << lane) - 1;
  int qn = 0, nq = 0;
  int dg[5] = {0, 0, 0, 0, 0};
  for (int64_t base = wlo; base < whi; base += int64_t(F) * kWave) {
    int tt[F];
    unsigned sk[F];
    an.restart();
    an.count(0);
#pragma unroll
    for (int u = 0; u < F; u++) {
      const int64_t row = base + u * kWave + lane;
      tt[u] = row < whi ? rtgt[row] : kRetired;
      sk[u] = row < whi ? unsigned(skey[row]) : 1u;
    }
    if (an.on()) {
      int ts = 0;
#pragma unroll
      for (int u = 0; u < F; u++)
        ts += tt[u] + int(sk[u]);
      an.level(6, ts);
    }
    bool ch[F];
#pragma unroll
    for (int u = 0; u < F; u++) {
      if (kBits)
        ch[u] = tt[u] >= 0 && ((bits[tt[u] >> 6] >> (tt[u] & 63)) & 1);
      else
        ch[u] = tt[u] >= 0 && s.chg[tt[u]] == prev;
    }
    unsigned kt[F], cg[F];
#pragma unroll
    for (int u = 0; u < F; u++) {
      kt[u] = ch[u] ? key[tt[u]] : 0u;
      cg[u] = (kBits && !ch[u] && tt[u] >= 0 && sk[u] == 0) ? unsigned(s.chg[tt[u]]) : 0x10000u;
    }
    if (an.on()) {
      unsigned ks = 0;
#pragma unroll
      for (int u = 0; u < F; u++)
        ks += kt[u] + cg[u];
      an.level(7, ks);
    }
    unsigned needm = 0;
#pragma unroll
    for (int u = 0; u < F; u++) {
      bool need = tt[u] == kUnvoted;
      if (ch[u])
        need = key_dead(kt[u]) || !(kt[u] < sk[u]);
      else if (kBits && cg[u] == prev)
        need = true;
      if (vm.sat_retire() && kDiag == 0 && ch[u] && kt[u] == kSatKey) {
        s.rtgt[buf][base + u * kWave + lane] = kRetired;
        need = false;
      }
      needm |= unsigned(need) << u;
      if (kDiag == 1) {
        dg[0] += ch[u];
        dg[1] += tt[u] >= 0 && sk[u] == 0;
        dg[2] += need;
        if (need && tt[u] >= 0) {
          atomicOr(reinterpret_cast<unsigned long long*>(&s.flagbits[tt[u] >> 6]), 1ull << (tt[u] & 63));
          dg[3] += sk[u] == 0;
        }
        dg[4] += ch[u] && kt[u] == kSatKey;
      }
    }
#pragma unroll 1
    for (int u = 0; u < F; u++) {
      const bool need = (needm >> u) & 1;
      const unsigned long long m = __ballot(need);
      if (need)
        qw[qn + __popcll(m & below)] = int(base + u * kWave + lane);
      qn += __popcll(m);
      if (qn >= kWave) {
        __builtin_amdgcn_wave_barrier();
        qn -= kWave;
        nq += kWave;
        const int row = qw[qn + lane];
        __builtin_amdgcn_wave_barrier();
        int pc = -1;
        an.restart();
        an.count(1);
        if (kDiag == 0)
          vote_row<R, M>(s, buf, round, row, st_rows, st_elems, key, &pc, ar);
        if (vm.rdq() && kDiag == 0)
          rdq_push_lds(s, pc, round, rql);
        an.level(8, 0u);
      }
    }
  }
  __builtin_amdgcn_wave_barrier();
  if (an.on() && qn > 0) {
    an.restart();
    an.count(1);
  }
  int pc = -1;
  if (kDiag == 0 && lane < qn)
    vote_row<R, M>(s, buf, round, qw[lane], st_rows, st_elems, key, &pc, ar);
  if (vm.rdq() && kDiag == 0)
    rdq_push_lds(s, pc, round, rql);
  if (an.on() && qn > 0)
    an.level(8, 0u);
  if (kDiag == 1 && s.vstat && round < kStatRounds) {
    int32_t* d = s.vstat + 2 * (int64_t(round) * kMaxBlocks + kDiagSlot);
    for (int k = 0; k < 5; k++) {
      const int t = grp_isum<kWave>(dg[k]);
      if (lane == 0 && t)
        atomicAdd(&d[k == 3 ? 6 : k == 4 ? 7 : k], t);
    }
  }
  return nq + qn;
}

constexpr int kBitWords = 17408;

#ifndef LMM_BITS_UNROLL
#define LMM_BITS_UNROLL 2
#endif
#ifndef LMM_BITS_STAGGER
#define LMM_BITS_STAGGER 1
#endif
template <int B, bool kStagger = false, int kU = 1>
__device__ __forceinline__ void load_bits(const Dev& s, uint64_t* bits) {
  const int n16 = (s.nC + 127) / 128;
  const uint4* __restrict__ src = reinterpret_cast<const uint4*>(s.chgbits);
  uint4* dst = reinterpret_cast<uint4*>(bits);
  const int off = kStagger && n16 > 0 ? int((int64_t(blockIdx.x) * 4099 * B) % n16) : 0;
  for (int i0 = threadIdx.x; i0 < n16; i0 += kU * B) {
    uint4 t[kU];
#pragma unroll
    for (int u = 0; u < kU; u++)
      if (i0 + u * B < n16) {
        const int i = kStagger ? (i0 + u * B + off) % n16 : i0 + u * B;
        t[u] = src[i];
      }
#pragma unroll
    for (int u = 0; u < kU; u++)
      if (i0 + u * B < n16) {
        const int i = kStagger ? (i0 + u * B + off) % n16 : i0 + u * B;
        dst[i] = t[u];
      }
  }
}

__global__ void __launch_bounds__(kBlock) mm_vote_diagcount(Dev s, int round) {
  int nf = 0, deg = 0;
  for (int64_t w = int64_t(blockIdx.x) * kBlock + threadIdx.x; w < (s.nC + 63) / 64; w += int64_t(gridDim.x) * kBlock) {
    unsigned long long m = s.flagbits[w];
    s.flagbits[w] = 0;
    while (m) {
      const int b = __ffsll((long long)m) - 1;
      m &= m - 1;
      const int64_t c = w * 64 + b;
      nf++;
      deg += int(s.cnst_ptr[c + 1] - s.cnst_ptr[c]);
    }
  }
  nf = grp_isum<kWave>(nf);
  deg = grp_isum<kWave>(deg);
  if ((threadIdx.x & (kWave - 1)) == 0 && s.vstat && round < kStatRounds) {
    int32_t* d = s.vstat + 2 * (int64_t(round) * kMaxBlocks + kDiagSlot);
    atomicAdd(&d[4], nf);
    atomicAdd(&d[5], deg);
  }
}

constexpr int kVBlock = vote_block(VoteForm::Bitmap);
template <VoteForm V, int M, int kDiag = 0>
__global__ void __launch_bounds__(vote_block(V)) mm_vote_lane(Dev s, int round) {
  constexpr int B = vote_block(V);
  constexpr bool kBits = vote_bits(V), kRdq = vote_mode(M).rdq();
  AnatWave aw, awr;
  const Anat an = kDiag == 0 ? aw.open(s, round, ANAT_VOTE) : Anat();
  const Anat ar = kDiag == 0 ? awr.open(s, round, ANAT_VOTE) : Anat();
  const unsigned long long t_in = an.now();
  if (s.ctl[CTL_DONE])
    return;
  const int buf = s.ctl[CTL_BUF];
  __shared__ int st_rows, st_elems;
  __shared__ int q[(B / kWave) * kQW];
  __shared__ __attribute__((aligned(16))) uint64_t bits[kBits ? kBitWords : 2];
  __shared__ RdqLds rql;
  if (threadIdx.x == 0) {
    st_rows = st_elems = 0;
    rql.n = 0;
  }
  const int64_t nrows = s.ctl[CTL_NROWS + buf];
  const int64_t per = ((nrows + gridDim.x - 1) / gridDim.x + kWave - 1) / kWave * kWave;
  const int64_t lo = int64_t(blockIdx.x) * per;
  const int64_t hi = lo + per < nrows ? lo + per : nrows;
  if (kBits)
    load_bits<B, LMM_BITS_STAGGER != 0, LMM_BITS_UNROLL>(s, bits);
  __syncthreads();
  const unsigned long long t_bits = an.now();
  if (kDiag == 2) {
    if (kBits && blockIdx.x == 0 && s.vstat && round < kStatRounds) {
      int pc = 0;
      for (int i = threadIdx.x; i < (s.nC + 63) / 64; i += B)
        pc += __popcll(bits[i]);
      atomicAdd(s.vstat + 2 * (int64_t(round) * kMaxBlocks + kDiagSlot) + 3, pc);
    }
    if (threadIdx.x == 0 && bits[1] == 0x5a5a5a5a5a5a5a5aull)
      s.ctl[CTL_WORDS - 1] = 1;
    return;
  }
  int nq = 0;
  if (lo < hi)
    nq = vote_waves<kBits, 8, kFilt, kDiag, M>(s, buf, round, lo, hi, bits, q + (threadIdx.x / kWave) * kQW, &st_rows,
                                               &st_elems, s.key, &rql, an, ar);
  if (kRdq && kDiag == 0)
    rdq_flush_lds(s, round, &rql);
  if (an.on()) {
    const unsigned long long t_out = an.now();
    unsigned lv[6];
#pragma unroll
    for (int i = 0; i < 6; i++)
      lv[i] = anat_wmax(ar.lv(i));
    int64_t wlo, whi;
    vote_wave_range(lo, hi, wlo, whi);
    if ((threadIdx.x & (kWave - 1)) == 0) {
      an.put(0, t_in);
      an.put(1, t_out);
      an.put(2, blockIdx.x);
      an.put(3, t_bits);
      an.put(4, an.cnt(0));
      an.put(5, an.lv(6));
      an.put(6, an.lv(7));
      an.put(7, an.cnt(1));
      an.put(8, an.lv(8));
#pragma unroll
      for (int i = 0; i < 6; i++)
        an.put(9 + i, lv[i]);
      an.put(15, unsigned(nq));
      an.put(16, whi > wlo ? unsigned(whi - wlo) : 0u);
    }
  }
  if (s.vstat && kDiag == 0) {
    __syncthreads();
    if (threadIdx.x == 0 && round < kStatRounds && blockIdx.x < kMaxBlocks) {
      s.vstat[2 * (int64_t(round) * kMaxBlocks + blockIdx.x)] = st_rows;
      s.vstat[2 * (int64_t(round) * kMaxBlocks + blockIdx.x) + 1] = st_elems;
    }
  }
}

__device__ __forceinline__ int64_t chunk_of(int64_t n, int nblocks) { return (n + nblocks - 1) / nblocks; }

__global__ void __launch_bounds__(kBlock) mm_ready(Dev s) {
  if (s.ctl[CTL_DONE])
    return;
  const int cb = s.ctl[CTL_CB];
  __shared__ int cnt;
  if (threadIdx.x == 0)
    cnt = 0;
  __syncthreads();
  const int64_t n = s.ctl[CTL_NCL0 + cb];
  const int64_t chunk = chunk_of(n, gridDim.x);
  const int64_t lo = int64_t(blockIdx.x) * chunk;
  const int64_t hi = lo + chunk < n ? lo + chunk : n;
  for (int64_t i = lo + threadIdx.x; i < hi; i += kBlock) {
    const int32_t c = s.clist[cb][i];
    if (!key_dead(s.key[c]) && s.nvote[c] == 0)
      s.ready[lo + atomicAdd(&cnt, 1)] = c;
  }
  __syncthreads();
  if (threadIdx.x == 0)
    s.bready[blockIdx.x] = cnt;
}



#ifndef LMM_KSATU
#define LMM_KSATU 4
#endif
constexpr int kSatU = LMM_KSATU;

__device__ __forceinline__ void saturate_chunk(const Dev& s, int32_t c, double r, uint32_t j0, uint32_t ce,
                                               int round, int lane, int* pre, bool dup, Anat an = Anat()) {
  an.restart();
  an.count(1);
  const int q = lane & 3;
  const uint32_t j = j0 + lane;
  int32_t lv = -1;
  double lp = 1.0, lx = 0.0;
  uint32_t rb = 0, re = 0;
  if (j < ce) {
    lv = s.csc_v[j];
    lp = s.csc_p[j];
    const unsigned long long row = s.csc_row[j];
    rb = uint32_t(row);
    re = uint32_t(row >> 32);
  }
// ... 325 lines not shown
    if (i >= total)
      return q[i - total];
    int lo = 0;
#pragma unroll
    for (int step = kMaxBlocks / 2; step > 0; step >>= 1)
      if (lo + step < ublocks && pre[lo + step] <= i)
        lo += step;
    return s.useg[int64_t(lo) * kUSeg + (i - pre[lo])];
  };
  struct CandSt {
    int32_t c;
    unsigned kc;
    int nv;
    double r;
    uint32_t cb, ce;
    bool dup;
  };
  auto state_of = [&](int32_t c) -> CandSt {
    CandSt x;
    x.c = c;
    if (c < 0) {
      x.kc = kDeadKey;
      x.nv = 1;
      x.r = 0.0;
      x.cb = x.ce = 0;
      x.dup = false;
      return x;
    }
    x.kc = s.key[c];
    x.nv = s.nvote[c];
    x.r = ld_rlx(&s.cst[c].ratio);
    x.cb = s.cnst_ptr[c];
    x.ce = s.cnst_ptr[c + 1];
    x.dup = s.cdup[c] != 0;
    return x;
  };
  CandSt cur = state_of(wave < T ? cand_of(wave) : -1);
  int32_t cnext = wave + nwaves < T ? cand_of(wave + nwaves) : -1;
  for (int64_t g = wave; g < T; g += nwaves) {
    const int k = int(g % K);
    an.restart();
    an.count(0);
    an.level(6, cur.r + double(cur.kc + unsigned(cur.nv) + cur.cb + cur.ce + unsigned(cur.dup)));
    const CandSt nxt = state_of(cnext);
    cnext = g + 2 * nwaves < T ? cand_of(g + 2 * nwaves) : -1;
    if (!key_dead(cur.kc) && cur.nv == 0) {
      saturate_one_pre<K>(s, cur.c, k, round, lane, wpre[w], cur.r, cur.cb, cur.ce, cur.dup, an);
    }
    cur = nxt;
  }
  if (an.on() && lane == 0) {
    an.put(0, t_in);
    an.put(1, an.now());
    an.put(2, blockIdx.x);
    an.put(3, t_pre);
    for (int f = 0; f < 7; f++)
      an.put(4 + f, an.lv(f));
    for (int f = 0; f < 4; f++)
      an.put(11 + f, an.cnt(f));
  }
}

using u32x4 = uint32_t __attribute__((ext_vector_type(4)));
union UpdPiece {
  u32x4 v;
  unsigned long long q[2];
};
template <int K> struct UpdQuadLds {
  static_assert(kWave == 64, "16 quads x 4 passes cover a group; owner lanes are 6-bit (& 63)");
  UpdPiece tile[4][kWave];
  uint32_t own[K][kWave / 4];
  static_assert(sizeof(own[0]) == kWave, "one byte per rank of a group");
  __device__ __forceinline__ void set_owner(int k, int r, int lane) {
    reinterpret_cast<unsigned char*>(own[k])[4 * (r & 15) + (r >> 4)] = (unsigned char)lane;
  }
};
__device__ __forceinline__ void wave_lds_sync() {
  __builtin_amdgcn_fence(__ATOMIC_RELEASE, "wavefront");
  __builtin_amdgcn_wave_barrier();
  __builtin_amdgcn_fence(__ATOMIC_ACQUIRE, "wavefront");
}
template <int K, int U>
__device__ __forceinline__ int update_groups(const Dev& s, int64_t wbase, int64_t stride, int round, double prec,
                                             bool* touch, int* ucnt_sh = nullptr, int32_t* ulist = nullptr,
                                             Anat an = Anat(), UpdQuadLds<K>* ql = nullptr) {
  static_assert(upd_mode_ok(U), "not an update mode");
  constexpr bool kRdq = upd_mode(U).rdq(), kQuad = upd_mode(U).quad();
  const int lane = threadIdx.x & (kWave - 1);
  const int64_t base0 = kQuad ? int64_t(uint32_t(__builtin_amdgcn_readfirstlane(int(wbase)))) |
                                    int64_t(__builtin_amdgcn_readfirstlane(int(wbase >> 32))) << 32
                              : wbase;
  an.restart();
  an.count(0);
  unsigned okey[K], tf[K];
#pragma unroll
  for (int k = 0; k < K; k++) {
    const int64_t c = base0 + k * stride + lane;
    okey[k] = c < s.nC ? unsigned(s.key[c]) : kDeadKey;
    tf[k] = c < s.nC ? unsigned(s.ctouch[c]) : 0u;
  }
  if (an.on()) {
    unsigned ks = 0;
#pragma unroll
    for (int k = 0; k < K; k++)
      ks += okey[k] + tf[k];
    an.level(0, ks);
  }
  unsigned long long qx[K], qy[K], qz[K];
  double rem[K], use[K], bnd[K];
  int32_t ce[K], nv[K];
  unsigned long long tm[kQuad ? K : 1], sm[kQuad ? K : 1];
  uint32_t ow[kQuad ? K : 1];
  u32x4 pc[kQuad ? K : 1][4];
  const int qr = lane >> 2, qp = lane & 3;
  if constexpr (!kQuad) {
#pragma unroll
    for (int k = 0; k < K; k++) {
      const int64_t c = base0 + k * stride + lane;
      qx[k] = qy[k] = qz[k] = 0;
      rem[k] = use[k] = bnd[k] = 0.0;
      ce[k] = nv[k] = 0;
      if (!key_dead(okey[k]) && tf[k] == 1) {
        const CstRec* rec = s.cst + c;
        qx[k] = rec->drem;
        qy[k] = rec->duse;
        qz[k] = rec->dcnt;
        rem[k] = rec->rem;
        use[k] = rec->use;
        bnd[k] = rec->bound;
        ce[k] = s.cexp[c];
        nv[k] = s.nvote[c];
      }
    }
  } else {
    const unsigned long long below = (1ull << lane) - 1;
#pragma unroll
    for (int k = 0; k < K; k++) {
      const bool t = !key_dead(okey[k]) && tf[k] == 1;
      tm[k] = __ballot(t);
      sm[k] = __ballot(!key_dead(okey[k]) && tf[k] == 2);
      if (t)
        ql->set_owner(k, __popcll(tm[k] & below), lane);
    }
    wave_lds_sync();
#pragma unroll
    for (int k = 0; k < K; k++)
      ow[k] = ql->own[k][qr];
#pragma unroll
    for (int k = 0; k < K; k++) {
      const int64_t gbase = base0 + k * stride;
      const int n = __popcll(tm[k]);
      ce[k] = nv[k] = 0;
      if ((tm[k] >> lane) & 1) {
        ce[k] = s.cexp[gbase + lane];
        nv[k] = s.nvote[gbase + lane];
      }
#pragma unroll
      for (int p = 0; p < 4; p++)
        if (16 * p + qr < n)
          pc[k][p] = reinterpret_cast<const u32x4*>(s.cst + (gbase + ((ow[k] >> (8 * p)) & 63)))[qp];
    }
  }
  if (an.on()) {
    double rs = 0.0;
#pragma unroll
    for (int k = 0; k < K; k++) {
      if constexpr (!kQuad) {
// ... 32 lines not shown
      rem[k] = use[k] = bnd[k] = 0.0;
      if (tch) {
        const u32x4 a = ql->tile[0][lane].v, b = ql->tile[1][lane].v, d = ql->tile[2][lane].v, e = ql->tile[3][lane].v;
        qx[k] = a.x | (unsigned long long)a.y << 32;
        qy[k] = a.z | (unsigned long long)a.w << 32;
        qz[k] = b.x | (unsigned long long)b.y << 32;
        rem[k] = __longlong_as_double((long long)(d.x | (unsigned long long)d.y << 32));
        use[k] = __longlong_as_double((long long)(d.z | (unsigned long long)d.w << 32));
        bnd[k] = __longlong_as_double((long long)(e.z | (unsigned long long)e.w << 32));
      }
    }
    const bool fat = tch && (ce[k] & kCexpFat);
    const bool fre = fat && !(__longlong_as_double((long long)qy[k]) < use[k]);
    double fuse = use[k];
    unsigned long long fm = __ballot(fre);
    while (fm) {
      const int l = __ffsll((long long)fm) - 1;
      fm &= fm - 1;
      const int64_t cl = gbase + l;
      const uint32_t b = s.cnst_ptr[cl], e = s.cnst_ptr[cl + 1];
      double m = 0.0;
      for (uint32_t j = b + lane; j < e; j += kWave) {
        const double u = s.csc_u[j];
        m = !(s.x[s.csc_v[j]] > 0) ? fmax(m, u) : m;
      }
      m = wave_max(m);
      if (lane == l)
        fuse = m;
    }
    bool changed = false;
    CstRec* rec = s.cst + c;
    double wr = 0.0, wu = 0.0, wq = 0.0;
    if (sat) {
      *touch = true;
      s.key[c] = kSatKey;
      s.cexp[c] = kCexpDead;
      s.chg[c] = uint16_t(round);
      s.ctouch[c] = 0;
      rec->ratio = dinf();
      changed = true;
    } else if (live) {
      if (!tch) {
        alive++;
      } else {
        *touch = true;
        s.ctouch[c] = 0;
        if constexpr (!kQuad)
          rec->drem = rec->duse = rec->dcnt = 0;
        const int nvn = nv[k] - int(qz[k]);
        s.nvote[c] = nvn;
        s.chg[c] = uint16_t(round);
        double r0 = rem[k], u0;
        if (!fat) {
          u0 = use[k] - dec_val(qy[k], cexp_use(ce[k]));
          r0 -= dec_val(qx[k], cexp_rem(ce[k]));
          if (r0 < bnd[k] * prec)
            r0 = 0.0;
          if (u0 < prec)
            u0 = 0.0;
        } else {
          u0 = fuse;
        }
        if constexpr (!kQuad) {
          rec->rem = r0;
          rec->use = u0;
        } else {
          wr = r0;
          wu = u0;
        }
        if (!(u0 > prec) || !(r0 > bnd[k] * prec)) {
          if constexpr (!kQuad)
            rec->ratio = dinf();
          else
            wq = dinf();
          s.key[c] = kDeadKey;
          s.cexp[c] = kCexpDead;
          changed = true;
        } else {
          const double r = r0 / u0;
          if constexpr (!kQuad)
            rec->ratio = r;
          else
            wq = r;
          const unsigned nk = ratio_key(r);
          s.key[c] = uint16_t(nk);
          changed = nk != okey[k];
          alive++;
          if (kRdq && nvn == 0) {
            const int slot = atomicAdd(ucnt_sh, 1);
            ulist[slot] = int32_t(c);
            s.rqst[c] = round + 1;
          }
        }
      }
    }
    if constexpr (kQuad) {
      if (tch) {
        const unsigned long long br = (unsigned long long)__double_as_longlong(wr);
        const unsigned long long bu = (unsigned long long)__double_as_longlong(wu);
        const unsigned long long bq = (unsigned long long)__double_as_longlong(wq);
        ql->tile[0][lane].v = u32x4{0u, 0u, 0u, 0u};
        ql->tile[1][lane].q[0] = 0ull;
        ql->tile[2][lane].v = u32x4{uint32_t(br), uint32_t(br >> 32), uint32_t(bu), uint32_t(bu >> 32)};
        ql->tile[3][lane].q[0] = bq;
      }
      wave_lds_sync();
      const int n = __popcll(tm[k]);
      const uint32_t o4 = ql->own[k][qr];
#pragma unroll
      for (int p = 0; p < 4; p++)
        if (16 * p + qr < n) {
          const int o = (o4 >> (8 * p)) & 63;
          reinterpret_cast<u32x4*>(s.cst + (gbase + o))[qp] = ql->tile[qp][o].v;
        }
      wave_lds_sync();
    }
    const unsigned long long word = __ballot(changed);
    if (lane == 0)
      s.chgbits[gbase >> 6] = word;
  }
  an.level(2, alive);
  return alive;
}

#ifndef LMM_UPD_K
#define LMM_UPD_K 4
#endif
template <int U>
__global__ void __launch_bounds__(kBlock, upd_mode(U).quad() ? 4 : 1) mm_update(Dev s, int round, double prec) {
  constexpr bool kRdq = upd_mode(U).rdq(), kQuad = upd_mode(U).quad();
  AnatWave aw;
  const Anat an = aw.open(s, round, ANAT_UPD);
  const unsigned long long t_in = an.now();
  if (s.ctl[CTL_DONE])
    return;
  if (blockIdx.x == 0 && threadIdx.x == 0)
    s.ctl[CTL_ROUNDS] += 1;
  __shared__ int alive_cnt, ucnt_sh;
  __shared__ int32_t ulist[kRdq ? kUSeg : 1];
  __shared__ std::conditional_t<kQuad, UpdQuadLds<LMM_UPD_K>, int> qlds[kBlock / kWave];
  UpdQuadLds<LMM_UPD_K>* ql = nullptr;
  if constexpr (kQuad)
    ql = &qlds[threadIdx.x / kWave];
  if (threadIdx.x == 0)
    alive_cnt = ucnt_sh = 0;
  __syncthreads();
  int alive = 0;
  bool any_touch = false;
  const int64_t stride = int64_t(gridDim.x) * kBlock;
  for (int64_t base = (int64_t(blockIdx.x) * kBlock + threadIdx.x) & ~int64_t(kWave - 1); base < s.nC;
       base += LMM_UPD_K * stride)
    alive += update_groups<LMM_UPD_K, U>(s, base, stride, round, prec, &any_touch, &ucnt_sh, ulist, an, ql);
  const unsigned long long t_loop = an.now();
  if (alive)
    atomicAdd(&alive_cnt, alive);
  __syncthreads();
  if (threadIdx.x == 0)
    s.balive[blockIdx.x] = alive_cnt;
  if (kRdq) {
    const int n = ucnt_sh;
    for (int i = threadIdx.x; i < n; i += kBlock)
      s.useg[int64_t(blockIdx.x) * kUSeg + i] = ulist[i];
    if (threadIdx.x == 0)
      s.ucnt[blockIdx.x] = n;
  }
  if (__syncthreads_or(any_touch) && threadIdx.x == 0)
    s.ctl[CTL_LASTR] = round;
  if (an.on() && (threadIdx.x & (kWave - 1)) == 0) {
    an.put(0, t_in);
    an.put(1, an.now());
    an.put(2, blockIdx.x);
    an.put(3, t_loop);
    for (int f = 0; f < 3; f++)
      an.put(4 + f, an.lv(f));
    an.put(7, an.cnt(0));
    an.put(8, an.cnt(1));
  }
}

__global__ void __launch_bounds__(kBlock) mm_done(Dev s, int update_blocks) {
  int a = 0;
  for (int b = threadIdx.x; b < update_blocks; b += kBlock)
    a += s.balive[b];
  a = grp_isum<kWave>(a);
  __shared__ int w[kBlock / kWave];
  if ((threadIdx.x & (kWave - 1)) == 0)
    w[threadIdx.x / kWave] = a;
  __syncthreads();
  if (threadIdx.x == 0 && w[0] + w[1] + w[2] + w[3] == 0)
    s.ctl[CTL_DONE] = 1;
}


__device__ __forceinline__ void block_scan2(int& a, int& b, int* sh) {
  const int t = threadIdx.x;
  sh[t] = a;
  sh[kBlock + t] = b;
  __syncthreads();
  for (int o = 1; o < kBlock; o <<= 1) {
    int xa = t >= o ? sh[t - o] : 0, xb = t >= o ? sh[kBlock + t - o] : 0;
    __syncthreads();
    sh[t] += xa;
    sh[kBlock + t] += xb;
    __syncthreads();
  }
  a = sh[t] - a;
  b = sh[kBlock + t] - b;
  __syncthreads();
}

__device__ __forceinline__ bool row_alive(const Dev& s, int in, int64_t row) {
  return s.vstate[rvar(s.cvar[in][row])] == 0;
}

__global__ void __launch_bounds__(kBlock) cmp_count(Dev s) {
  if (s.ctl[CTL_DONE])
    return;
  const int in = s.ctl[CTL_BUF];
  __shared__ int sh[2 * kBlock];
  const int64_t nrows = s.ctl[CTL_NROWS + in];
  const int64_t r0 = int64_t(blockIdx.x) * kCompactRows + int64_t(threadIdx.x) * kRowsPerThread;
  int32_t cv[kRowsPerThread];
#pragma unroll
  for (int k = 0; k < kRowsPerThread; k++)
    cv[k] = r0 + k < nrows ? s.cvar[in][r0 + k] : -1;
  bool al[kRowsPerThread];
  uint32_t rb[kRowsPerThread + 1];
#pragma unroll
  for (int k = 0; k < kRowsPerThread; k++)
    al[k] = r0 + k < nrows && s.vstate[rvar(cv[k])] == 0;
#pragma unroll
  for (int k = 0; k <= kRowsPerThread; k++)
    rb[k] = r0 + k <= nrows ? s.crow[in][r0 + k] : 0u;
  int nr = 0, ne = 0;
#pragma unroll
  for (int k = 0; k < kRowsPerThread; k++)
    if (al[k]) {
      nr++;
      ne += int(rb[k + 1] - rb[k]);
    }
  int a = nr, b = ne;
  block_scan2(a, b, sh);
  if (threadIdx.x == kBlock - 1) {
    s.bsum[2 * blockIdx.x] = a + nr;
    s.bsum[2 * blockIdx.x + 1] = b + ne;
  }
}

__global__ void __launch_bounds__(kBlock) cmp_count_rows(Dev s, uint8_t* __restrict__ alive) {
  static_assert(kRowsPerThread == 8, "one byte of alive bits per thread");
  if (s.ctl[CTL_DONE])
    return;
  const int in = s.ctl[CTL_BUF];
  __shared__ int sh[2 * kBlock];
  const int64_t nrows = s.ctl[CTL_NROWS + in];
  const int64_t base = int64_t(blockIdx.x) * kCompactRows + threadIdx.x;
  const uint4* __restrict__ rec = s.crec[in].r16;
  uint4 rr[kRowsPerThread];
#pragma unroll
// ... 213 lines not shown
```

### simgrid_amd/csrc/lmm_persist_kernels.hpp

```cpp
#pragma once
#include "lmm_maxmin_kernels.hpp"

namespace lmmdev {

constexpr int kPB = 1024;
constexpr int kPW = kPB / kWave;
constexpr int kPBitWords = 16384;
constexpr int kPFilt = 4;
constexpr long long kSpinTicks = 400000000;

enum : int {
  BAR_XCNT = 0,
  BAR_TOP = 128,
  BAR_GEN = 144,
  BAR_XGEN = 160,
  BAR_XSIZE = 288,
  BAR_FLAT = 416,
  BAR_ALLOC = 432,
  BAR_PALIVE = 448,
  BAR_WORDS = 480
};

__device__ __forceinline__ unsigned xcc_id() {
  unsigned v;
// ... 70 lines not shown
    }
    ok_sh = ok;
  }
  __syncthreads();
  return ok_sh;
}

__device__ bool grid_sync(const PBar& b, unsigned gen) {
  __shared__ int ok_sh;
  asm volatile("s_waitcnt vmcnt(0)" ::: "memory");
  __syncthreads();
  if (threadIdx.x == 0) {
    int ok = 1;
    if (b.pt && gen < b.pt_cap) {
      const long long now = wall_clock64();
      atomicMax(&b.pt[2 * gen], now);
      if (gen < kPBlkCap)
        b.pt[2 * b.pt_cap + 2 * (size_t(gen) * gridDim.x + blockIdx.x)] = now;
    }
    const unsigned a =
        __hip_atomic_fetch_add(&b.w[BAR_XCNT + 16 * b.xcc], 1u, __ATOMIC_RELAXED, __HIP_MEMORY_SCOPE_AGENT);
    if (a == gen * b.xsize - 1) {
      if (b.sysf)
        __builtin_amdgcn_fence(__ATOMIC_RELEASE, "");
      else
        __builtin_amdgcn_fence(__ATOMIC_RELEASE, "agent");
      asm volatile("s_waitcnt vmcnt(0)" ::: "memory");
      const unsigned t = __hip_atomic_fetch_add(&b.w[BAR_TOP], 1u, __ATOMIC_RELAXED, __HIP_MEMORY_SCOPE_AGENT);
      if (t == gen * b.nx - 1)
        st_rlx(&b.w[BAR_GEN], gen);
      else
        ok = spin_geq(&b.w[BAR_GEN], gen, b.err);
      if (ok)
        st_rlx(&b.w[BAR_XGEN + 16 * b.xcc], gen);
    } else {
      ok = spin_geq(&b.w[BAR_XGEN + 16 * b.xcc], gen, b.err);
    }
    if (b.sysf)
      __builtin_amdgcn_fence(__ATOMIC_ACQUIRE, "");
    else
      __builtin_amdgcn_fence(__ATOMIC_ACQUIRE, "agent");
    asm volatile("s_waitcnt vmcnt(0)" ::: "memory");
    if (b.pt && gen < b.pt_cap) {
      const long long now = wall_clock64();
      if (blockIdx.x == 0)
        b.pt[2 * gen + 1] = now;
      if (gen < kPBlkCap)
        b.pt[2 * b.pt_cap + 2 * (size_t(gen) * gridDim.x + blockIdx.x) + 1] = now;
    }
    ok_sh = ok;
  }
  __syncthreads();
  return ok_sh;
}

__device__ __forceinline__ int64_t pwave() { return int64_t(threadIdx.x / kWave) * gridDim.x + blockIdx.x; }

template <bool kBits> struct PVoteLds {
  uint64_t bits[kBits ? kPBitWords : 2];
  int q[kPW * kQW];
  int st0, st1;
};
using PSatLds = SatLds<kPB, 4 * kPB>;
template <bool kBits> union PLds {
  PVoteLds<kBits> v;
  PSatLds sat;
  int pre[kPW][kWave];
  int cnt;
};

template <bool kBits, int R>
__device__ void p_vote(const Dev& s, int buf, int round, int64_t nrows, PVoteLds<kBits>& L, bool count) {
  if (threadIdx.x == 0)
    L.st0 = 0;
  if (kBits)
    load_bits<kPB>(s, L.bits);
  __syncthreads();
  const int64_t per = ((nrows + gridDim.x - 1) / gridDim.x + kWave - 1) / kWave * kWave;
  const int64_t lo = int64_t(blockIdx.x) * per;
  const int64_t hi = lo + per < nrows ? lo + per : nrows;
  int nq = 0;
  if (lo < hi)
    nq = vote_waves<kBits, R, kPFilt, 0, kVoteArrays>(s, buf, round, lo, hi, L.bits,
                                                      L.q + (threadIdx.x / kWave) * kQW, &L.st0, &L.st1, s.key);
  if (count) {
    if ((threadIdx.x & (kWave - 1)) == 0 && nq)
      atomicAdd(&L.st0, nq);
    __syncthreads();
    if (threadIdx.x == 0 && L.st0)
      atomicAdd(&s.ctl[CTL_RESEVAL], L.st0);
  }
}

__device__ void p_saturate(const Dev& s, int round, PSatLds& L) { sat_block<kPB, 4 * kPB>(s, round, nullptr, s.nC, L); }

__device__ void p_compact(const Dev& s, int in, int out, int64_t nrows, unsigned long long* alloc, int* sh) {
  const int lane = threadIdx.x & (kWave - 1), w = threadIdx.x / kWave;
  int32_t* ovar = const_cast<int32_t*>(s.cvar[out]);
  uint32_t* orow = const_cast<uint32_t*>(s.crow[out]);
  int32_t* ocol = const_cast<int32_t*>(s.ccol[out]);
  const int64_t per = ((nrows + gridDim.x - 1) / gridDim.x + kPB - 1) / kPB * kPB;
  const int64_t lo = int64_t(blockIdx.x) * per;
  const int64_t hi = lo + per < nrows ? lo + per : nrows;
  int nr = 0, ne = 0;
  for (int64_t row = lo + threadIdx.x; row < hi; row += kPB)
    if (s.vstate[rvar(s.cvar[in][row])] == 0) {
      nr++;
      ne += int(s.crow[in][row + 1] - s.crow[in][row]);
    }
  nr = grp_isum<kWave>(nr);
  ne = grp_isum<kWave>(ne);
  if (lane == 0) {
    sh[2 * w] = nr;
    sh[2 * w + 1] = ne;
  }
  __syncthreads();
  if (threadIdx.x == 0) {
    unsigned long long tr = 0, te = 0;
    for (int i = 0; i < kPW; i++) {
      tr += unsigned(sh[2 * i]);
      te += unsigned(sh[2 * i + 1]);
    }
    const unsigned long long old = tr ? atomicAdd(alloc, (tr << 32) | te) : 0ull;
    sh[2 * kPW] = int(old >> 32);
    sh[2 * kPW + 1] = int(uint32_t(old));
    sh[2 * kPW + 2] = tr != 0;
  }
  __syncthreads();
  uint32_t rbase = uint32_t(sh[2 * kPW]), ebase = uint32_t(sh[2 * kPW + 1]);
  const bool allocated = sh[2 * kPW + 2] != 0;
  __syncthreads();
  for (int64_t b0 = lo; b0 < hi; b0 += kPB) {
    const int64_t row = b0 + threadIdx.x;
    int32_t v = 0;
    bool al = false;
    uint32_t b = 0, e = 0;
    if (row < hi) {
      v = s.cvar[in][row];
      al = s.vstate[rvar(v)] == 0;
      if (al) {
        b = s.crow[in][row];
        e = s.crow[in][row + 1];
      }
    }
    int xr = al, xe = int(e - b);
    int ir = xr, ie = xe;
#pragma unroll
    for (int o = 1; o < kWave; o <<= 1) {
      const int tr = __shfl_up(ir, o, kWave), te = __shfl_up(ie, o, kWave);
      if (lane >= o) {
        ir += tr;
        ie += te;
      }
    }
    if (lane == kWave - 1) {
      sh[2 * w] = ir;
      sh[2 * w + 1] = ie;
    }
    __syncthreads();
    int orr = 0, oe = 0, tr = 0, te = 0;
    for (int i = 0; i < kPW; i++) {
      orr += i < w ? sh[2 * i] : 0;
      oe += i < w ? sh[2 * i + 1] : 0;
      tr += sh[2 * i];
      te += sh[2 * i + 1];
    }
    if (al) {
      const uint32_t o = rbase + uint32_t(orr + ir - xr);
      const uint32_t dst = ebase + uint32_t(oe + ie - xe);
      ovar[o] = v;
      s.rtgt[out][o] = s.rtgt[in][row];
      s.skey[out][o] = s.skey[in][row];
      orow[o] = dst;
      for (int j = 0; j < xe; j++)
        ocol[dst + j] = s.ccol[in][b + j];
    }
    rbase += uint32_t(tr);
    ebase += uint32_t(te);
    __syncthreads();
  }
  if (threadIdx.x == 0 && allocated)
    orow[rbase] = ebase;
}

template <bool kBits, int R>
__global__ void __launch_bounds__(kPB) mm_persist(Dev s, unsigned* barw, double prec, int max_rounds,
                                                  int cmp_every, long long* pt, unsigned pt_cap, int sysf,
                                                  long long rdv_ticks, int32_t* hflag) {
  __shared__ PLds<kBits> L;
  PBar b{barw, &s.ctl[CTL_ERR], 0, 0, 0, pt, pt_cap, sysf};
  if (pt && blockIdx.x == 0 && threadIdx.x == 0)
    pt[1] = wall_clock64();
  unsigned long long* alloc = reinterpret_cast<unsigned long long*>(barw + BAR_ALLOC);
  int32_t* palive = reinterpret_cast<int32_t*>(barw + BAR_PALIVE);
  const int lane = threadIdx.x & (kWave - 1);
  const bool lead = blockIdx.x == 0 && threadIdx.x == 0;
  if (!bar_rdv(b, rdv_ticks, hflag))
    return;
  unsigned gen = 0;
  init_cnsts_waves(s, nullptr, prec, pwave(), int64_t(gridDim.x) * kPW);
  init_vars_range<RowForm::Arrays>(s, int64_t(blockIdx.x) * kPB + threadIdx.x, int64_t(gridDim.x) * kPB);
  if (!grid_sync(b, ++gen))
    return;
  int buf = 0;
  int64_t nrows = s.nV;
  for (int r = 0;; r++) {
    p_vote<kBits, R>(s, buf, r, nrows, L.v, pt != nullptr);
    if (!grid_sync(b, ++gen))
      return;
    if (lead) {
      for (int i = 0; i < 8; i++)
        st_rlx(&palive[16 * ((r + 1) & 1) + i], 0);
      st_rlx(alloc, 0ull);
    }
    p_saturate(s, r, L.sat);
    if (!grid_sync(b, ++gen))
      return;
    if (threadIdx.x == 0)
      L.cnt = 0;
    __syncthreads();
    {
      int alive = 0;
      bool touch = false;
      constexpr int kU = 3;
      const int64_t stride = int64_t(gridDim.x) * kPB;
      for (int64_t base = pwave() * kWave; base < s.nC; base += kU * stride)
        alive += update_groups<kU, kUpdPlain>(s, base, stride, r, prec, &touch);
      alive = grp_isum<kWave>(alive);
      if (lane == 0 && alive)
        atomicAdd(&L.cnt, alive);
    }
    __syncthreads();
    if (threadIdx.x == 0 && L.cnt)
      atomicAdd(&palive[16 * (r & 1) + (blockIdx.x & 7)], L.cnt);
    if (!grid_sync(b, ++gen))
      return;
    int alive_all = 0;
    for (int i = 0; i < 8; i++)
      alive_all += ld_rlx(&palive[16 * (r & 1) + i]);
    if (alive_all == 0) {
      if (lead) {
        s.ctl[CTL_ROUNDS] = r + 1;
        s.ctl[CTL_LASTR] = r;
      }
      return;
    }
    if (r + 1 >= max_rounds) {
      if (lead)
        st_rlx(&s.ctl[CTL_ERR], 2);
      return;
    }
    if (cmp_every > 0 && r % cmp_every == cmp_every - 1 && nrows > kPB) {
      const int out = buf == 1 ? 2 : 1;
      p_compact(s, buf, out, nrows, alloc, &L.pre[0][0]);
      if (!grid_sync(b, ++gen))
        return;
      nrows = int64_t(ld_rlx(alloc) >> 32);
      buf = out;
    }
  }
}

}
```

### simgrid_amd/csrc/lmm_round_mode.hpp

```cpp
#pragma once
#include <algorithm>
#include <cstdint>

enum class RowForm { Arrays, Rec8, Rec16 };

enum class VoteForm { Bitmap, Scan };
constexpr int vote_block(VoteForm f) { return f == VoteForm::Bitmap ? 1024 : 256; }
constexpr bool vote_bits(VoteForm f) { return f == VoteForm::Bitmap; }

constexpr int kVoteModes = 9;
struct VoteMode {
  RowForm form = RowForm::Arrays;
  bool queue = false;
  bool filter = false;
  constexpr bool rec() const { return form != RowForm::Arrays; }
  constexpr bool rec16() const { return form == RowForm::Rec16; }
  constexpr bool rdq() const { return queue; }
  constexpr bool sat_retire() const { return filter; }
  constexpr bool tie_loads() const { return rec(); }
  constexpr bool valid() const { return rec() || (!queue && !filter); }
  constexpr int index() const { return !rec() ? 0 : 1 + 4 * int(rec16()) + 2 * int(queue) + int(filter); }
};
constexpr VoteMode vote_mode(int i) {
  return i == 0 ? VoteMode{} : VoteMode{(i - 1) & 4 ? RowForm::Rec16 : RowForm::Rec8, ((i - 1) & 2) != 0, ((i - 1) & 1) != 0};
}
constexpr bool vote_mode_ok(int i) {
  return i >= 0 && i < kVoteModes && vote_mode(i).valid() && vote_mode(i).index() == i;
}
constexpr int kVoteArrays = 0;

constexpr int kUpdModes = 4;
struct UpdMode {
  bool queue = false, quad4 = false;
  constexpr bool rdq() const { return queue; }
  constexpr bool quad() const { return quad4; }
  constexpr int index() const { return 2 * int(queue) + int(quad4); }
};
constexpr UpdMode upd_mode(int i) { return UpdMode{(i & 2) != 0, (i & 1) != 0}; }
constexpr bool upd_mode_ok(int i) { return i >= 0 && i < kUpdModes; }
constexpr int kUpdPlain = 0;

struct RoundKnobs {
  int crec = 1, rdq = 1, satkey = 1, cmp_rows = 1, upd_quad = 1, upd_blocks = 0, updq_blocks = 0;
};
constexpr int updq_blocks_default(int n_cu) { return 4 * n_cu; }
struct RoundLimits {
  int block, useg, max_blocks;
};
struct RoundMode {
  VoteMode vote;
  bool upd_quad = false;
  bool rdq_fits = false;
  int g_upd = 1;
  constexpr UpdMode upd() const { return UpdMode{vote.queue, upd_quad}; }
};

constexpr int64_t round_grid_for(int64_t n, int per_block, int max_blocks) {
  return std::max<int64_t>(1, std::min<int64_t>((n + per_block - 1) / per_block, max_blocks));
}

constexpr RoundMode resolve_round_mode(int group, int64_t nC, const RoundKnobs& k, const RoundLimits& L) {
  RoundMode m;
  const bool rec = (group == 4 || group == 8) && k.crec != 0;
  const int64_t g_c = round_grid_for(nC, L.block, L.max_blocks);
  const int64_t g_need = (nC + L.useg - 1) / L.useg;
  const int64_t g_rdq = std::max<int64_t>(1, std::min<int64_t>(g_c, std::max<int64_t>(g_need, k.updq_blocks)));
  const int64_t per_blk = int64_t(L.block) * ((nC + g_rdq * L.block - 1) / (g_rdq * L.block));
  m.rdq_fits = per_blk <= L.useg && k.upd_blocks == 0;
  m.vote.form = !rec ? RowForm::Arrays : k.cmp_rows != 0 ? RowForm::Rec16 : RowForm::Rec8;
  m.vote.queue = rec && k.rdq != 0 && m.rdq_fits;
  m.vote.filter = rec && k.satkey != 0;
  m.upd_quad = k.upd_quad != 0;
  m.g_upd = int(m.vote.queue ? g_rdq : k.upd_blocks > 0 && g_c > k.upd_blocks ? k.upd_blocks : g_c);
  return m;
}
```

### simgrid_amd/lmm.py

```python
import ctypes as ct
import os

import numpy as np

_HERE = os.path.dirname(os.path.abspath(__file__))
LIB_PATH = os.path.join(_HERE, "_lib", "liblmm_amd.so")
LIB_PATH = os.environ.get("LMM_AMD_LIB") or LIB_PATH

P, D, I, I64, U64 = ct.c_void_p, ct.c_double, ct.c_int, ct.c_int64, ct.c_uint64
PI, PD, PI64 = ct.POINTER(I), ct.POINTER(D), ct.POINTER(I64)

FAT_TREE, DRAGONFLY = 0, 1
SHARED, SPLITDUPLEX, FATPIPE = 0, 1, 2
CM02, LV08, L07 = 0, 1, 2


class PlatformParams(ct.Structure):
    _fields_ = [("topology", I), ("topo_parameters", ct.c_char_p), ("bw", D), ("lat", D), ("policy", I),
                ("loopback_bw", D), ("loopback_lat", D), ("limiter_bw", D), ("speed", D), ("model", I),
                ("crosstraffic", I), ("n_flows", I64), ("seed", U64), ("size_min", D), ("size_max", D),
                ("tcp_gamma", D)]


def platform_params(topology=FAT_TREE, topo_parameters="", bw=1.25e8, lat=5e-5, policy=SPLITDUPLEX, loopback_bw=0.0,
# ... 65 lines not shown
    "lmm_variable_rank": (I, [P, I64]),
    "lmm_variable_number_of_constraints": (I, [P, I64]),
    "lmm_get_values": (I, [P, PI64, I64, PD]),
    "lmm_system_variables": (I, [P, PI64, I]),
    "lmm_system_active_constraints": (I, [P, PI64, I]),
    "lmm_modified_actions": (I, [P, PI64, I]),
    "lmm_clear_modified_actions": (I, [P]),
    "lmm_expand": (I, [P, I64, I64, D]),
    "lmm_expand_add": (I, [P, I64, I64, D]),
    "lmm_update_variable_bound": (I, [P, I64, D]),
    "lmm_update_variable_penalty": (I, [P, I64, D]),
    "lmm_update_constraint_bound": (I, [P, I64, D]),
    "lmm_solve": (I, [P]),
    "lmm_lmm_solve": (I, [P]),
    "lmm_is_modified": (I, [P]),
    "lmm_prepare": (I, [P]),
    "lmm_device_solve": (I, [P]),
    "lmm_fetch": (I, [P]),
    "lmm_last_stats": (I, [P, PI64, PD]),
    "lmm_set_resident": (I, [P, I]),
    "lmm_is_resident": (I, [P]),
    "lmm_pending_deltas": (I, [P, PI64]),
    "lmm_last_delta_records": (ct.c_int64, [P]),
    "lmm_table_sizes": (I, [P, PI64]),
    "lmm_resident_drain": (I, [P, PI64, PI64, ct.POINTER(ct.c_int32), PD, ct.POINTER(ct.c_uint8), ct.POINTER(ct.c_int32), PI64, ct.POINTER(ct.c_int32), PD, PD, ct.POINTER(ct.c_int32), PD, ct.POINTER(ct.c_uint8)]),
    "lmm_flat_export": (I, [P, PI64, PI64, ct.POINTER(ct.c_int32), PD, PD, PD, PD, ct.POINTER(ct.c_uint8), PI64]),
    "lmm_flat_export_order": (I, [P, I64, PI64]),
    "lmm_flat_export_cnsts": (I, [P, PI64, I64]),
    "lmm_device_usage": (I64, [P, PI64, PD, I64]),
    "lmm_device_certificate": (I, [P, D, PD, PI64, PI64]),
    "lmm_device_bottlenecks": (I64, [P, PI64, PI64, I64]),
    "lmm_solve_batch": (I, [ct.POINTER(P), I]),
    "lmm_system_device_ctx": (P, [P]),
    "lmm_check_certificate": (I, [P, D, PD, PI64, PI64]),
    "lmm_gen_maxmin_bench": (I, [P, I, I, PI64, PI64, PI, PI]),
    "lmm_gen_synthetic": (I64, [P, I64, I64, I, U64, I, I, I, I, PI64]),
    "lmm_platform_size": (I, [ct.POINTER(PlatformParams), PI64, PI64]),
    "lmm_platform_dragonfly_coords": (I64, [ct.POINTER(PlatformParams), ct.POINTER(ct.c_int32), I64]),
    "lmm_gen_platform_flows": (I64, [P, ct.POINTER(PlatformParams), PI64, PI64]),
    "lmm_link_new": (I64, [P, I, D, I]),
    "lmm_communicate": (I64, [P, P, I, I64, PI64, PD, PD, I64, PI64, D, D, I, P]),
    "lmm_wifi_link_new": (I64, [P, I]),
    "lmm_communicate_ex": (I64, [P, P, I, I64, PI64, PD, PD, PD, I64, PI64, I, D, D, I, P]),
    "lmm_device_count": (I, []),
    "lmm_last_error": (ct.c_char_p, []),
    "lmmhip_ctx_create": (I, [I, ct.POINTER(P)]),
    "lmmhip_ctx_destroy": (I, [P]),
    "lmmhip_upload": (I, [P, I64, I64, I64, PI64, ct.POINTER(ct.c_int32), PD, PD, PD, PD, ct.POINTER(ct.c_uint8)]),
    "lmmhip_upload2": (I, [P, I64, I64, I64, PI64, ct.POINTER(ct.c_int32), PD, PD, PD, PD, ct.POINTER(ct.c_uint8),
                           PI64]),
    "lmmhip_update_vars": (I, [P, PD, PD]),
    "lmmhip_update_cnsts": (I, [P, PD]),
    "lmmhip_res_apply": (I, [P, I64, I64, I64, I64, PI64, ct.POINTER(ct.c_int32), PD, ct.POINTER(ct.c_uint8), I64, ct.POINTER(ct.c_int32), PI64, ct.POINTER(ct.c_int32), PD, PD, I64, ct.POINTER(ct.c_int32), PD, ct.POINTER(ct.c_uint8)]),
    "lmmhip_res_flatten": (I, [P, I64, ct.POINTER(ct.c_int32), D, PI64]),
    "lmmhip_res_values": (I, [P, I64, PD, ct.POINTER(ct.c_uint8)]),
    "lmmhip_res_flatten_fair": (I, [P, I64, ct.POINTER(ct.c_int32), PI64]),
    "lmmhip_res_values_pinned": (I, [P, I64, ct.POINTER(P), ct.POINTER(P)]),
    "lmmhip_res_values_sliced": (I, [P, I64, I, ct.POINTER(P)]),
    "lmmhip_res_values_wait": (I, [P, I]),
    "lmmhip_res_refreshes": (I, [P, PI64]),
    "lmmhip_res_cross_refreshes": (I, [P, PI64]),
    "lmmhip_flat_download": (I, [P, PI64, P, P, P, P, P, P, P, P, P, P]),
    "lmmhip_solve": (I, [P, I, D]),
    "lmmhip_set_batch": (I, [P, I64, PI64, PI64]),
    "lmmhip_get_values": (I, [P, PD]),
    "lmmhip_get_var_rounds": (I, [P, ct.POINTER(ct.c_int32)]),
    "lmmhip_values_device_ptr": (I, [P, ct.POINTER(P)]),
    "lmmhip_get_saturated": (I, [P, ct.POINTER(ct.c_uint8)]),
    "lmmhip_get_touched_vars": (I, [P, ct.POINTER(ct.c_int32), I64, PI64]),
    "lmmhip_get_usage": (I, [P, PD]),
    "lmmhip_usage_device_ptr": (I, [P, ct.POINTER(P)]),
    "lmmhip_get_touched_cnsts": (I, [P, ct.POINTER(ct.c_int32), I64, PI64]),
    "lmmhip_certificate": (I, [P, D, ct.POINTER(LmmhipCert), ct.POINTER(ct.c_int32)]),
    "lmmhip_get_stats": (I, [P, P]),
    "lmmhip_set_profiling": (I, [P, I]),
    "lmmhip_launch_profile": (I, [P, PI, PI, ct.POINTER(ct.c_float), I]),
    "lmmhip_round_profile": (I, [P, PI64, PI64, I]),
    "lmmhip_vote_profile": (I, [P, PI64, PI64, I]),
    "lmmhip_vote_diag_profile": (I, [P, PI64, I]),
    "lmmhip_ctx_set_stream": (I, [P, P]),
    "lmmhip_ctx_use_own_stream": (I, [P]),
    "lmmhip_ctx_set_engine": (I, [P, I]),
    "lmmhip_engine_fallbacks": (I, [P, PI64]),
    "lmmhip_last_engine": (I, [P, PI]),
    "lmmhip_persist_profile": (I, [P, I, PI64, I64, PI64]),
    "lmmhip_persist_profile_blocks": (I, [P, PI64, I64, PI64, PI64]),
    "lmmhip_fb_shard_owner": (I, [P, I64, ct.POINTER(ct.c_int32), PI64, ct.POINTER(ct.c_int32), PD,
                                  ct.POINTER(ct.c_int32), I64, I64]),
    "lmmhip_fb_shard_begin": (I, [P, D, P, P, I64, P]),
    "lmmhip_fb_shard_step": (I, [P, I]),
    "lmmhip_fb_shard_pack_mu": (I, [P, P, P, P]),
    "lmmhip_fb_shard_poll": (I, [P, PI, PI64]),
    "lmmhip_fb_work": (I, [P, PI64]),
    "lmmhip_components": (I, [P, PI, PI, PI64]),
    "lmmhip_actions_upload": (I, [P, I64, ct.POINTER(ct.c_int32), PD, PD, PD, PD, PD, ct.POINTER(ct.c_uint8)]),
    "lmmhip_next_event_full": (I, [P, I, PD]),
    "lmmhip_update_actions_full": (I, [P, I, D, D, D, PI64]),
    "lmmhip_actions_download": (I, [P, PD, PD, PD, PD, ct.POINTER(ct.c_uint8)]),
    "lmmhip_actions_lazy_upload": (I, [P, PD, PD, PD, PD, ct.POINTER(ct.c_uint8)]),
    "lmmhip_actions_lazy_update": (I, [P, I, D, D, D, I64, ct.POINTER(ct.c_int32), PI64]),
    "lmmhip_next_event_lazy": (I, [P, D, PD]),
    "lmmhip_actions_lazy_due": (I, [P, I, D, D, ct.POINTER(ct.c_int32), ct.POINTER(ct.c_uint8), I64, PI64]),
    "lmmhip_actions_lazy_download": (I, [P, PD, PD, PD, ct.POINTER(ct.c_uint8)]),
    "lmmhip_actions_bind": (I, [P, I64, ct.POINTER(ct.c_int32)]),
    "lmmhip_actions_patch": (I, [P, I64, ct.POINTER(ct.c_int32), I, ct.POINTER(ct.c_int32), PD, PD, PD, PD, PD,
                                 ct.POINTER(ct.c_uint8), PD, PD, PD, PD, ct.POINTER(ct.c_uint8)]),
    "lmmhip_actions_lazy_update_solved": (I, [P, I, D, D, D, I64, ct.POINTER(ct.c_int32), PI64, PI64]),
    "lmmhip_actions_events": (I, [P, ct.POINTER(ct.c_int32), ct.POINTER(ct.c_uint8), I64, PI64]),
    "lmmhip_actions_var_index": (I, [P, ct.POINTER(ct.c_int32)]),
    "lmmhip_device_count": (I, []),
    "lmmhip_last_error": (ct.c_char_p, []),
    "lmmhip_build_id": (ct.c_char_p, []),
    "lmmhip_anatomy": (I, [P, ct.POINTER(ct.c_uint64), I64, PI64, ct.POINTER(ct.c_int32)]),
}

_lib = None


class LmmError(RuntimeError):
    pass


def _missing_symbol(name):
    def stub(*_a, **_k):
        raise LmmError(f"{name} not exported by the LMM_AMD_LIB build ({LIB_PATH})")
    return stub


def lib():
    global _lib
    if _lib is None:
        try:
            import torch
        except Exception:
            pass
        if not os.path.exists(LIB_PATH):
            raise LmmError(f"{LIB_PATH} is missing: build it with `python -c 'import __graft_entry__ as g; g.build()'`")
        l = ct.CDLL(LIB_PATH)
        for name, (res, args) in SIGNATURES.items():
            f = getattr(l, name, None)
            if f is None and os.environ.get("LMM_AMD_LIB"):
                setattr(l, name, _missing_symbol(name))
                continue
            if f is None:
                raise LmmError(f"{LIB_PATH} does not export {name}: rebuild it")
            f.restype = res
            f.argtypes = args
        _lib = l
    return _lib


def _check(rc):
    if rc != 0:
        raise LmmError(lib().lmm_last_error().decode())
    return rc


def _check_hip(rc):
    if rc != 0:
        raise LmmError(lib().lmmhip_last_error().decode())
    return rc


def build_id():
    return lib().lmmhip_build_id().decode()

# ... 182 lines not shown
    def device_solve(self):
        _check(lib().lmm_device_solve(self.h))

    def fetch(self):
        _check(lib().lmm_fetch(self.h))

    def last_stats(self):
        c, m = (I64 * 4)(), (D * 4)()
        lib().lmm_last_stats(self.h, c, m)
        return dict(rounds=c[0], n_var=c[1], n_cnst=c[2], nnz=c[3], device_ms=m[0], flatten_ms=m[1],
                    upload_ms=m[2], fetch_ms=m[3], delta_records=lib().lmm_last_delta_records(self.h))

    def components(self):
        self.prepare()
        st = self.last_stats()
        return ctx_components(self.device_ctx(), st["n_var"], st["n_cnst"])

    def fb_work(self):
        w = (I64 * 3)()
        _check_hip(lib().lmmhip_fb_work(self.device_ctx(), w))
        return w[0], w[1], w[2]

    def set_resident(self, on=True):
        _check(lib().lmm_set_resident(self.h, int(bool(on))))

    def resident(self):
        return bool(lib().lmm_is_resident(self.h))

    def drain_deltas(self):
        ne, nv, nc = self.pending_deltas()
        sz = (I64 * 6)(ne, nv, nc, 0, 0, 0)
        if min(ne, nv, nc) < 0:
            _check(lib().lmm_table_sizes(self.h, sz))
        a = dict(e_id=np.zeros(sz[0], np.int64), e_cnst=np.zeros(sz[0], np.int32), e_w=np.zeros(sz[0]),
                 e_fl=np.zeros(sz[0], np.uint8), v_id=np.zeros(sz[1], np.int32), v_eb=np.zeros(sz[1], np.int64),
                 v_n=np.zeros(sz[1], np.int32), v_p=np.zeros(sz[1]), v_b=np.zeros(sz[1]),
                 c_id=np.zeros(sz[2], np.int32), c_b=np.zeros(sz[2]), c_fl=np.zeros(sz[2], np.uint8))
        ptr = lambda x: x.ctypes.data_as(ct.POINTER(np.ctypeslib.as_ctypes_type(x.dtype)))
        _check(lib().lmm_resident_drain(self.h, sz, *(ptr(a[k]) for k in (
            "e_id", "e_cnst", "e_w", "e_fl", "v_id", "v_eb", "v_n", "v_p", "v_b", "c_id", "c_b", "c_fl"))))
        n = dict(e=sz[0], v=sz[1], c=sz[2])
        out = {k: v[:n[k[0]]] for k, v in a.items()}
        out["totals"] = (sz[3], sz[4], sz[5])
        return out

    def device_flat(self):
        ctx = self.device_ctx()
        n = (I64 * 3)()
        _check_hip(lib().lmmhip_flat_download(ctx, n, *([None] * 10)))
        nV, nC, nnz = n
        a = dict(var_ptr=np.zeros(nV + 1, np.uint32), csr_c=np.zeros(nnz, np.int32), csr_w=np.zeros(nnz),
                 cnst_ptr=np.zeros(nC + 1, np.uint32), csc_v=np.zeros(nnz, np.int32), csc_w=np.zeros(nnz),
                 pen=np.zeros(nV), vbound=np.zeros(nV), cbound=np.zeros(nC), cflags=np.zeros(nC, np.uint8))
        _check_hip(lib().lmmhip_flat_download(ctx, n, *(x.ctypes.data for x in a.values())))
        return a

    def pending_deltas(self):
        o = (I64 * 3)()
        _check(lib().lmm_pending_deltas(self.h, o))
        return tuple(o)

    def check_certificate(self, precision=None):
        ex, ni, nu = D(), I64(), I64()
        p = get_precision() if precision is None else precision
        _check(lib().lmm_check_certificate(self.h, p, ct.byref(ex), ct.byref(ni), ct.byref(nu)))
        return ex.value, ni.value, nu.value

    def device_ctx(self):
        c = lib().lmm_system_device_ctx(self.h)
        if not c:
            raise LmmError(lib().lmm_last_error().decode())
        return c

    ENGINE_PERSISTENT, ENGINE_ROUNDS, ENGINE_AUTO, ENGINE_FRONTIER = 0, 1, 2, 3

    def set_engine(self, engine):
        _check_hip(lib().lmmhip_ctx_set_engine(self.device_ctx(), int(engine)))

    def engine_fallbacks(self):
        n = ct.c_int64()
        _check_hip(lib().lmmhip_engine_fallbacks(self.device_ctx(), ct.byref(n)))
        return n.value

    RAN_PERSISTENT, RAN_ROUNDS, RAN_FRONTIER, RAN_BATCH, RAN_FB_ROUNDS, RAN_FB_BATCH = range(6)

    def last_engine(self):
        e = I()
        _check_hip(lib().lmmhip_last_engine(self.device_ctx(), ct.byref(e)))
        return e.value

    def device_values(self):
        n = self.last_stats()["n_var"]
        x = np.empty(n, np.float64)
        _check_hip(lib().lmmhip_get_values(self.device_ctx(), x.ctypes.data_as(PD)))
        return x

    def device_var_rounds(self):
        n = self.last_stats()["n_var"]
        r = np.empty(n, np.int32)
        _check_hip(lib().lmmhip_get_var_rounds(self.device_ctx(), r.ctypes.data_as(ct.POINTER(ct.c_int32))))
        return r

    def device_saturated(self):
        out = np.empty(self.last_stats()["n_cnst"], np.uint8)
        _check_hip(lib().lmmhip_get_saturated(self.device_ctx(), out.ctypes.data_as(ct.POINTER(ct.c_uint8))))
        return out.astype(bool)

    def device_usage_dense(self):
        out = np.empty(self.last_stats()["n_cnst"], np.float64)
        _check_hip(lib().lmmhip_get_usage(self.device_ctx(), out.ctypes.data_as(PD)))
        return out

    def device_usage(self):
        n = lib().lmm_device_usage(self.h, None, None, 0)
        if n < 0:
            raise LmmError(lib().lmm_last_error().decode())
        ids, u = np.empty(n, np.int64), np.empty(n, np.float64)
        if lib().lmm_device_usage(self.h, ids.ctypes.data_as(PI64), u.ctypes.data_as(PD), n) != n:
            raise LmmError(lib().lmm_last_error().decode())
        return ids, u

    def device_certificate(self, precision=None):
        ex, ni, nu = D(), I64(), I64()
        p = get_precision() if precision is None else precision
        _check(lib().lmm_device_certificate(self.h, p, ct.byref(ex), ct.byref(ni), ct.byref(nu)))
        return ex.value, ni.value, nu.value

    def device_certificate_dense(self, precision=None):
        p = get_precision() if precision is None else precision
        return ctx_certificate(self.device_ctx(), self.last_stats()["n_var"], p)

    def device_bottlenecks(self):
        n = lib().lmm_device_bottlenecks(self.h, None, None, 0)
        if n < 0:
            raise LmmError(lib().lmm_last_error().decode())
        vs, cs = np.empty(n, np.int64), np.empty(n, np.int64)
        if lib().lmm_device_bottlenecks(self.h, vs.ctypes.data_as(PI64), cs.ctypes.data_as(PI64), n) != n:
            raise LmmError(lib().lmm_last_error().decode())
        return vs, cs

    def flat_cnst_ids(self):
        cnt = (I64 * 3)()
        _check(lib().lmm_flat_export(self.h, cnt, None, None, None, None, None, None, None, None))
        ids = np.empty(cnt[1], np.int64)
        _check(lib().lmm_flat_export_cnsts(self.h, ids.ctypes.data_as(PI64), len(ids)))
        return ids

    def device_touched_vars(self):
        n = I64()
        ctx = self.device_ctx()
        _check_hip(lib().lmmhip_get_touched_vars(ctx, None, 0, ct.byref(n)))
        out = np.empty(n.value, np.int32)
        _check_hip(lib().lmmhip_get_touched_vars(ctx, out.ctypes.data_as(ct.POINTER(ct.c_int32)), n.value,
                                                 ct.byref(n)))
        return out

    def persist_profile(self, on=True):
        ctx = self.device_ctx()
        n = I64()
        cap = 1 << 17
        t = np.zeros(cap, np.int64)
        _check_hip(lib().lmmhip_persist_profile(ctx, int(on), t.ctypes.data_as(PI64), cap, ct.byref(n)))
        return t[:2 * n.value].reshape(-1, 2)

    def persist_profile_blocks(self):
        ctx = self.device_ctx()
# ... 166 lines not shown
```

Measured before the change: 464.9 million.

## Adapt 16-bit ratio keys to the observed ratio range and bound-key voting

Replaces the fixed-mantissa 16-bit ratio key with a per-solve window (base and shift) computed from the min and max initial constraint ratios, reduced across blocks in the init kernels. The goal is finer key resolution, so fewer ties force exact double-ratio scans. Variable bounds are also converted to keys, so bounded rows can be decided from keys alone. The cost is an extra reduction and key rewrite pass at init, plus clamping risk when ratios grow past the headroom factor.

```diff
diff --git a/include/lmm/lmm_hip.h b/include/lmm/lmm_hip.h
--- a/include/lmm/lmm_hip.h
+++ b/include/lmm/lmm_hip.h
@@ -98,6 +98,7 @@
 #define LMMHIP_ENGINE_FRONTIER 3
 int lmmhip_ctx_set_engine(lmmhip_ctx* ctx, int engine);
 int lmmhip_engine_fallbacks(lmmhip_ctx* ctx, int64_t* n);
+int lmmhip_key_window(lmmhip_ctx* ctx, int64_t* out);
 #define LMMHIP_RAN_PERSISTENT 0
 #define LMMHIP_RAN_ROUNDS 1
 #define LMMHIP_RAN_FRONTIER 2
diff --git a/simgrid_amd/csrc/lmm_ctx.hpp b/simgrid_amd/csrc/lmm_ctx.hpp
--- a/simgrid_amd/csrc/lmm_ctx.hpp
+++ b/simgrid_amd/csrc/lmm_ctx.hpp
@@ -109,6 +109,7 @@
 struct RoundEngine {
   Scr crec[3], rdq[2], rqst, useg, ucnt;
   Scr cmpbits;
+  Scr kwmm;
 };
 using VoteKernel = void (*)(Dev, int);
 using SatKernel = void (*)(Dev, int, int);
@@ -125,6 +126,8 @@
   int g_upd = 1;
   int cap_sat = 0, sat_max = 0;
   int cmp_every = 48, cmp_pct = 75, cl_every = 8;
+  bool key_window = true;
+  double key_headroom = 4.0;
   ChunkPolicy chunk;
   int64_t tail_rows = 0, tail_cnst = 0;
 };
diff --git a/simgrid_amd/csrc/lmm_dev.hpp b/simgrid_amd/csrc/lmm_dev.hpp
--- a/simgrid_amd/csrc/lmm_dev.hpp
+++ b/simgrid_amd/csrc/lmm_dev.hpp
@@ -6,6 +6,8 @@
 #include <climits>
 #include <cstdint>
 #include <type_traits>
+
+#include "lmm_keywin.hpp"
 
 namespace lmmdev {
 
@@ -35,6 +37,10 @@
   CTL_CB = 22,
   CTL_CMPGO = 23,
   CTL_FBW = 24,
+  CTL_KW_BASE = 25,
+  CTL_KW_SHIFT = 26,
+  CTL_KW_STORES = 27,
+  CTL_KW_CLAMP = 28,
   CTL_WORDS = 32
 };
 constexpr int kFbwSlots = 64;
@@ -245,12 +251,9 @@
 
 __device__ __forceinline__ double dinf() { return __builtin_huge_val(); }
 
-#ifndef LMM_KEY_MANT
-#define LMM_KEY_MANT 7
-#endif
-__device__ __forceinline__ uint16_t ratio_key(double r) {
-  float f = __double2float_rd(r);
-  return uint16_t(__float_as_uint(f) >> (23 - LMM_KEY_MANT));
+__device__ __forceinline__ uint16_t ratio_key(double r, KeyWin w) { return uint16_t(key_code(r, w)); }
+__device__ __forceinline__ KeyWin key_win_ctl(const int32_t* ctl) {
+  return KeyWin{uint32_t(ctl[CTL_KW_BASE]), ctl[CTL_KW_SHIFT]};
 }
 
 constexpr uint32_t kDead32 = 0xFFFFFFFFu;
diff --git a/simgrid_amd/csrc/lmm_frontier_kernels.hpp b/simgrid_amd/csrc/lmm_frontier_kernels.hpp
--- a/simgrid_amd/csrc/lmm_frontier_kernels.hpp
+++ b/simgrid_amd/csrc/lmm_frontier_kernels.hpp
@@ -81,12 +81,11 @@
 
 enum : int { FR_STAY = 0, FR_MOVE = 1, FR_BOUND = 2, FR_DROP = 3 };
 
-__device__ __forceinline__ uint32_t row_floor32(uint32_t sk, uint32_t mk, double vb, double p) {
-  uint32_t fl = sk;
-  if (vb > 0)
-    fl = min(fl, ratio_key32(vb * p));
+__device__ __forceinline__ uint32_t row_floor32(uint32_t sk, uint32_t mk, uint32_t kb) {
+  const uint32_t fl = min(sk, kb);
   return fl <= mk ? 0u : fl;
 }
+__device__ __forceinline__ uint32_t bound_key32(double vb, double p) { return vb > 0 ? ratio_key32(vb * p) : kDead32; }
 
 template <int R, bool kMinfl = true, bool kEarly = true>
 __device__ __forceinline__ int fr_revote(const FrDev& s, int v, int t, uint32_t b, uint32_t e, int round, Anat an) {
@@ -156,8 +155,10 @@
     if (k == mk)
       newt = min(newt, c);
   }
+  const uint32_t kb = bound_key32(vb, p);
+  const bool bfix = kb < mk;
   double minr = dinf();
-  if (nmin > 1 || vb > 0) {
+  if ((nmin > 1 && !bfix) || kb == mk) {
     newt = INT_MAX;
     double rr[R];
 #pragma unroll
@@ -181,7 +182,7 @@
     }
   }
   an.level(3, minr + double(newt + nmin));
-  if (vb > 0 && vb * p < minr) {
+  if (bfix || (kb == mk && vb * p < minr)) {
     s.vstate[v] = round + 1;
     s.x[v] = vb;
     if (t >= 0 && kt != kDead32)
@@ -214,7 +215,7 @@
       mfn = kNoVoter;
     }
   }
-  const uint32_t fl = min(row_floor32(sk, mk, vb, p), kNoVoter - 1u);
+  const uint32_t fl = min(row_floor32(sk, mk, kb), kNoVoter - 1u);
   if (kMinfl && !kEarly)
     mfn = s.minfl[newt];
   s.vslot[slot] = fl;
diff --git a/simgrid_amd/csrc/lmm_hip.hip b/simgrid_amd/csrc/lmm_hip.hip
--- a/simgrid_amd/csrc/lmm_hip.hip
+++ b/simgrid_amd/csrc/lmm_hip.hip
@@ -683,6 +683,18 @@
   return 0;
 }
 
+int lmmhip_key_window(lmmhip_ctx* c, int64_t* out) {
+  if (!c || !out)
+    return fail(LMMHIP_E_ARG, "null argument");
+  if (!c->solved || c->last_engine != LMMHIP_RAN_ROUNDS)
+    return fail(LMMHIP_E_STATE, "the last solve of this context did not run the round engine");
+  out[0] = int64_t(uint32_t(c->h_ctl.p[CTL_KW_BASE]));
+  out[1] = c->h_ctl.p[CTL_KW_SHIFT];
+  out[2] = c->h_ctl.p[CTL_KW_STORES];
+  out[3] = c->h_ctl.p[CTL_KW_CLAMP];
+  return 0;
+}
+
 int lmmhip_ctx_set_engine(lmmhip_ctx* c, int engine) {
   if (!c)
     return fail(LMMHIP_E_ARG, "null context");
diff --git a/simgrid_amd/csrc/lmm_hip_maxmin.hip b/simgrid_amd/csrc/lmm_hip_maxmin.hip
--- a/simgrid_amd/csrc/lmm_hip_maxmin.hip
+++ b/simgrid_amd/csrc/lmm_hip_maxmin.hip
@@ -12,6 +12,7 @@
 #include "lmm_frontier_kernels.hpp"
 #include "lmm_batch_kernels.hpp"
 
+constexpr double kKeyHeadroom = 4.0;
 constexpr int64_t kAutoPersistVars = 1 << 18;
 constexpr int64_t kAutoPersistMaxVars = 1 << 14;
 
@@ -105,6 +106,10 @@
   P.update = kUpdTable[m.upd().index()];
   P.g_init_c = grid_for(d.nC, kBlock / kWave);
   P.g_c = grid_for(d.nC, kBlock);
+  P.key_window = env_int("LMMHIP_KEY_WINDOW", 1) != 0;
+  const char* kh = std::getenv("LMMHIP_KEY_HEADROOM");
+  const double khv = kh ? std::atof(kh) : 0.0;
+  P.key_headroom = khv >= 1.0 ? khv : kKeyHeadroom;
   P.cmp_every = env_int("LMMHIP_COMPACT_EVERY", 48);
   P.cmp_pct = env_int("LMMHIP_COMPACT_PCT", 75);
   P.cl_every = env_int("LMMHIP_CLIST_EVERY", 8);
@@ -118,7 +123,10 @@
   return P;
 }
 
-static int round_buffers(lmmhip_ctx* c, Dev& d, const RoundPlan& P, uint8_t** cmpbits) {
+static int round_buffers(lmmhip_ctx* c, Dev& d, const RoundPlan& P, uint8_t** cmpbits, double** kwmm) {
+  if (P.key_window)
+    if (int rc = scratch(c, c->rounds.kwmm, 2 * int64_t(P.g_init_c), kwmm))
+      return rc;
   for (int k = 0; k < 3 && P.mode.rec(); k++)
     if (int rc = P.mode.rec16() ? scratch(c, c->rounds.crec[k], int64_t(d.nV) + 1, &d.crec[k].r16)
                                 : scratch(c, c->rounds.crec[k], int64_t(d.nV) + 1, &d.crec[k].r8))
@@ -155,10 +163,12 @@
   Dev d = c->d;
   const RoundPlan P = round_plan(c, d);
   uint8_t* cmpbits = nullptr;
-  if (int rc = round_buffers(c, d, P, &cmpbits))
-    return rc;
-  LAUNCH(0, -1, mm_init_cnsts, P.g_init_c, kBlock, d, static_cast<uint32_t*>(nullptr), prec);
-  LAUNCH(1, -1, mm_init_vars, grid_for(d.nV, kBlock), kBlock, d, int(P.mode.rec16()));
+  double* kwmm = nullptr;
+  if (int rc = round_buffers(c, d, P, &cmpbits, &kwmm))
+    return rc;
+  LAUNCH(0, -1, mm_init_cnsts, P.g_init_c, kBlock, d, static_cast<uint32_t*>(nullptr), prec, kwmm);
+  LAUNCH(1, -1, mm_init_vars, grid_for(d.nV, kBlock), kBlock, d, int(P.mode.rec16()), static_cast<const double*>(kwmm),
+         P.g_init_c, P.key_headroom);
   LAUNCH(1, -1, mm_clist, std::min(P.g_c, 2 * c->n_cu), kBlock, d, 1);
   HIPCHK(hipMemsetAsync(d.chgbits, 0, sizeof(uint64_t) * ((d.nC + 127) / 128 * 2 + 2), c->stream));
   int64_t last_compact = 0, last_clist = 0, nrows = d.nV, ncl = d.nC;
@@ -172,6 +182,8 @@
     LAUNCH(4, r, P.saturate, int(P.cap_sat > 0 && gS > P.cap_sat ? P.cap_sat : gS), kBlock, d, int(r),
            P.mode.rdq() ? P.g_upd : gL);
     LAUNCH(5, r, P.update, P.g_upd, kBlock, d, int(r), prec);
+    if (c->profiling && c->vote_diag)
+      LAUNCH(7, r, mm_key_diag, P.g_c, kBlock, d, int(r));
     return 0;
   };
   auto chunk_end = [&](int64_t r) -> int {
@@ -272,7 +284,7 @@
     c->frontier.map_ok = true;
   }
   const FrontierPlan P = frontier_plan(c, d);
-  LAUNCH(0, -1, mm_init_cnsts, grid_for(d.nC, kBlock / kWave), kBlock, d, d.key32, prec);
+  LAUNCH(0, -1, mm_init_cnsts, grid_for(d.nC, kBlock / kWave), kBlock, d, d.key32, prec, static_cast<double*>(nullptr));
   LAUNCH(1, -1, fr_init_vars, grid_for(std::max<int64_t>(std::max<int64_t>(d.nV, d.nC), d.nnz / 4), kBlock), kBlock, d);
   auto round_launches = [&](int64_t r) -> int {
     if (r == 0) {
diff --git a/simgrid_amd/csrc/lmm_keywin.hpp b/simgrid_amd/csrc/lmm_keywin.hpp
--- /dev/null
+++ b/simgrid_amd/csrc/lmm_keywin.hpp
@@ -0,0 +1,57 @@
+#pragma once
+#include <cmath>
+#include <cstdint>
+#include <cstring>
+
+#if defined(__HIPCC__)
+#define LMM_KW_FN __host__ __device__ __forceinline__
+#else
+#define LMM_KW_FN inline
+#endif
+
+#ifndef LMM_KEY_MANT
+#define LMM_KEY_MANT 7
+#endif
+
+struct KeyWin {
+  uint32_t base;
+  int shift;
+};
+constexpr unsigned kKeyTop = 0xFFFDu;
+constexpr KeyWin kKeyWinLegacy{0u, 23 - LMM_KEY_MANT};
+
+LMM_KW_FN uint32_t f32_rd_bits(double r) {
+#if defined(__HIP_DEVICE_COMPILE__)
+  return __float_as_uint(__double2float_rd(r));
+#else
+  float f = float(r);
+  if (double(f) > r)
+    f = std::nextafterf(f, -INFINITY);
+  uint32_t u;
+  std::memcpy(&u, &f, sizeof u);
+  return u;
+#endif
+}
+
+LMM_KW_FN unsigned key_code_bits(uint32_t bits, KeyWin w) {
+#if defined(__HIP_DEVICE_COMPILE__)
+  const uint32_t c = __builtin_elementwise_sub_sat(bits, w.base) >> w.shift;
+#else
+  const uint32_t c = ((bits > w.base ? bits : w.base) - w.base) >> w.shift;
+#endif
+  return c < kKeyTop ? unsigned(c) : kKeyTop;
+}
+LMM_KW_FN unsigned key_code(double r, KeyWin w) { return key_code_bits(f32_rd_bits(r), w); }
+
+LMM_KW_FN KeyWin key_window(double lo, double hi, double headroom) {
+  if (!(lo <= hi) || !(lo >= 0))
+    return kKeyWinLegacy;
+  KeyWin w;
+  w.base = f32_rd_bits(lo);
+  const uint32_t top = f32_rd_bits(hi * headroom);
+  const uint32_t span = top > w.base ? top - w.base : 0u;
+  w.shift = 0;
+  while ((span >> w.shift) > kKeyTop)
+    w.shift++;
+  return w;
+}
diff --git a/simgrid_amd/csrc/lmm_maxmin_kernels.hpp b/simgrid_amd/csrc/lmm_maxmin_kernels.hpp
--- a/simgrid_amd/csrc/lmm_maxmin_kernels.hpp
+++ b/simgrid_amd/csrc/lmm_maxmin_kernels.hpp
@@ -9,7 +9,7 @@
 
 constexpr int kInitG = 16;
 __device__ __forceinline__ int init_cnsts_waves(const Dev& s, uint32_t* key32, double prec, int64_t wave,
-                                                int64_t nwaves) {
+                                                int64_t nwaves, double& rlo, double& rhi) {
   const int lane = threadIdx.x & (kWave - 1), gl = lane & (kInitG - 1);
   constexpr int kGpw = kWave / kInitG;
   int alive_cnt = 0;
@@ -49,18 +49,72 @@
       s.cexp[c] = cexp_pack(alive ? dec_scale(bound) : 0, alive ? dec_scale(usage) : 0, fat, !alive);
       s.nvote[c] = int32_t(e - b);
       s.chg[c] = uint16_t(0xFFFF);
-      s.key[c] = alive ? ratio_key(r) : uint16_t(kDeadKey);
+      s.key[c] = alive ? ratio_key(r, kKeyWinLegacy) : uint16_t(kDeadKey);
       if (key32)
         key32[c] = alive ? ratio_key32(r) : kDead32;
+      rlo = alive ? fmin(rlo, r) : rlo;
+      rhi = alive ? fmax(rhi, r) : rhi;
       alive_cnt += alive;
     }
   }
   return alive_cnt;
 }
 
-__global__ void __launch_bounds__(kBlock) mm_init_cnsts(Dev s, uint32_t* key32, double prec) {
+__global__ void __launch_bounds__(kBlock) mm_init_cnsts(Dev s, uint32_t* key32, double prec, double* kwmm) {
   const int64_t wave = (int64_t(blockIdx.x) * kBlock + threadIdx.x) / kWave;
-  init_cnsts_waves(s, key32, prec, wave, int64_t(gridDim.x) * (kBlock / kWave));
+  double lo = dinf(), hi = 0.0;
+  init_cnsts_waves(s, key32, prec, wave, int64_t(gridDim.x) * (kBlock / kWave), lo, hi);
+  if (kwmm) {
+    __shared__ double wlo[kBlock / kWave], whi[kBlock / kWave];
+    lo = wave_min(lo);
+    hi = wave_max(hi);
+    if ((threadIdx.x & (kWave - 1)) == 0) {
+      wlo[threadIdx.x / kWave] = lo;
+      whi[threadIdx.x / kWave] = hi;
+    }
+    __syncthreads();
+    if (threadIdx.x == 0) {
+      for (int k = 1; k < kBlock / kWave; k++) {
+        lo = fmin(lo, wlo[k]);
+        hi = fmax(hi, whi[k]);
+      }
+      kwmm[2 * blockIdx.x] = lo;
+      kwmm[2 * blockIdx.x + 1] = hi;
+    }
+  }
+}
+
+__device__ __forceinline__ void key_window_pass(const Dev& s, const double* kwmm, int nslots, double headroom) {
+  KeyWin kw = kKeyWinLegacy;
+  if (kwmm) {
+    __shared__ double wlo[kBlock / kWave], whi[kBlock / kWave];
+    double lo = dinf(), hi = 0.0;
+    for (int i = threadIdx.x; i < nslots; i += kBlock) {
+      lo = fmin(lo, kwmm[2 * i]);
+      hi = fmax(hi, kwmm[2 * i + 1]);
+    }
+    lo = wave_min(lo);
+    hi = wave_max(hi);
+    if ((threadIdx.x & (kWave - 1)) == 0) {
+      wlo[threadIdx.x / kWave] = lo;
+      whi[threadIdx.x / kWave] = hi;
+    }
+    __syncthreads();
+    for (int k = 0; k < kBlock / kWave; k++) {
+      lo = fmin(lo, wlo[k]);
+      hi = fmax(hi, whi[k]);
+    }
+    kw = key_window(lo, hi, headroom);
+  }
+  if (blockIdx.x == 0 && threadIdx.x == 0) {
+    s.ctl[CTL_KW_BASE] = int32_t(kw.base);
+    s.ctl[CTL_KW_SHIFT] = kw.shift;
+  }
+  if (!kwmm)
+    return;
+  for (int64_t c = int64_t(blockIdx.x) * kBlock + threadIdx.x; c < s.nC; c += int64_t(gridDim.x) * kBlock)
+    if (!key_dead(s.key[c]))
+      s.key[c] = ratio_key(s.cst[c].ratio, kw);
 }
 
 template <RowForm F>
@@ -78,7 +132,9 @@
   }
 }
 
-__global__ void __launch_bounds__(kBlock) mm_init_vars(Dev s, int rec16) {
+__global__ void __launch_bounds__(kBlock) mm_init_vars(Dev s, int rec16, const double* kwmm, int nslots,
+                                                       double headroom) {
+  key_window_pass(s, kwmm, nslots, headroom);
   const int64_t t = int64_t(blockIdx.x) * kBlock + threadIdx.x, nthreads = int64_t(gridDim.x) * kBlock;
   if (rec16)
     init_vars_range<RowForm::Rec16>(s, t, nthreads);
@@ -126,11 +182,12 @@
     s.rdq[q][L->base + i] = L->buf[i];
 }
 
-__device__ __forceinline__ unsigned row_floor(unsigned sk, unsigned mk, double vb, double p) {
-  unsigned fl = sk;
-  if (vb > 0)
-    fl = min(fl, (unsigned)ratio_key(vb * p));
+__device__ __forceinline__ unsigned row_floor(unsigned sk, unsigned mk, unsigned kb) {
+  const unsigned fl = min(sk, kb);
   return fl <= mk ? 0u : fl;
+}
+__device__ __forceinline__ unsigned bound_key(double vb, double p, KeyWin kw) {
+  return vb > 0 ? unsigned(ratio_key(vb * p, kw)) : kDeadKey;
 }
 
 __device__ __forceinline__ unsigned long long fat_bits(double u) { return (unsigned long long)__double_as_longlong(u); }
@@ -156,6 +213,7 @@
   if (s.ctl[CTL_DONE])
     return;
   const int buf = s.ctl[CTL_BUF];
+  const KeyWin kw = key_win_ctl(s.ctl);
   __shared__ int st_rows, st_elems;
   if (s.vstat && threadIdx.x == 0)
     st_rows = st_elems = 0;
@@ -219,8 +277,11 @@
       nmin = grp_isum<G>(nmin);
       const double vb = need ? s.vbound[v] : -1.0;
       const bool live = need && !key_dead(mk);
+      const double p = need ? s.pen[v] : 1.0;
+      const unsigned kb = live ? bound_key(vb, p, kw) : kDeadKey;
+      const bool bfix = kb < mk;
       double minr = dinf();
-      if (live && (nmin > 1 || vb > 0)) {
+      if (live && ((nmin > 1 && !bfix) || kb == mk)) {
         if (h0 && k0 == mk)
           minr = s.cst[c0].ratio;
         for (uint32_t j = j0 + G; j < e; j += G) {
@@ -230,8 +291,7 @@
         }
       }
       minr = grp_min<G>(minr);
-      const double p = need ? s.pen[v] : 1.0;
-      const bool bounded = live && vb > 0 && vb * p < minr;
+      const bool bounded = live && (bfix || (kb == mk && vb * p < minr));
       int newt = INT_MAX;
       if (live && !bounded) {
         if (h0 && k0 == mk && (nmin == 1 || s.cst[c0].ratio == minr))
@@ -251,7 +311,7 @@
       }
       sk = grp_umin<G>(sk);
       if (live && !bounded && g == 0)
-        s.skey[buf][row] = uint16_t(row_floor(sk, mk, vb, p));
+        s.skey[buf][row] = uint16_t(row_floor(sk, mk, kb));
       int mult_new = h0 && c0 == newt, mult_old = h0 && c0 == t;
       for (uint32_t j = j0 + G; j < e; j += G) {
         const int32_t c = ccol[j];
@@ -362,8 +422,8 @@
 
 template <int R, int M>
 __device__ __forceinline__ void vote_row(const Dev& s, int buf, int round, int64_t row, int* st_rows,
-                                         int* st_elems, const uint16_t* __restrict__ key, int* rdq_c = nullptr,
-                                         Anat an = Anat()) {
+                                         int* st_elems, const uint16_t* __restrict__ key, KeyWin kw,
+                                         int* rdq_c = nullptr, Anat an = Anat()) {
   static_assert(vote_mode_ok(M), "not one of the nine vote modes");
   constexpr VoteMode vm = vote_mode(M);
   an.restart();
@@ -451,8 +511,11 @@
     if (k == mk)
       newt = min(newt, c);
   }
+  constexpr bool kBk = vm.bound_keys();
+  const unsigned kb = kBk ? bound_key(vb, p, kw) : kDeadKey;
+  const bool bfix = kBk && kb < mk;
   double minr = dinf();
-  if (nmin > 1 || vb > 0) {
+  if (kBk ? (nmin > 1 && !bfix) || kb == mk : nmin > 1 || vb > 0) {
     newt = INT_MAX;
     constexpr bool kTieLd = vm.tie_loads();
     double rr[kTieLd ? R : 1];
@@ -482,7 +545,7 @@
     }
   }
   an.level(4, minr + double(newt));
-  if (vb > 0 && vb * p < minr) {
+  if (bfix || ((kBk ? kb == mk : vb > 0) && vb * p < minr)) {
     s.vstate[v] = round + 1;
     s.x[v] = vb;
     rtgt[row] = kRetired;
@@ -508,7 +571,7 @@
       sk = min(sk, k);
     mult_new += c == newt;
   }
-  skey[row] = uint16_t(row_floor(sk, mk, vb, p));
+  skey[row] = uint16_t(row_floor(sk, mk, kBk ? kb : bound_key(vb, p, kw)));
   if (newt == t)
     return;
   if (t >= 0 && !key_dead(kt))
@@ -541,8 +604,8 @@
 template <bool kBits, int R, int F, int kDiag, int M>
 __device__ __forceinline__ int vote_waves(const Dev& s, int buf, int round, int64_t lo, int64_t hi,
                                           const uint64_t* bits, int* qw, int* st_rows, int* st_elems,
-                                          const uint16_t* __restrict__ key, RdqLds* rql = nullptr, Anat an = Anat(),
-                                          Anat ar = Anat()) {
+                                          const uint16_t* __restrict__ key, KeyWin kw, RdqLds* rql = nullptr,
+                                          Anat an = Anat(), Anat ar = Anat()) {
   constexpr VoteMode vm = vote_mode(M);
   const int lane = threadIdx.x & (kWave - 1);
   int64_t wlo, whi;
@@ -633,7 +696,7 @@
         an.restart();
         an.count(1);
         if (kDiag == 0)
-          vote_row<R, M>(s, buf, round, row, st_rows, st_elems, key, &pc, ar);
+          vote_row<R, M>(s, buf, round, row, st_rows, st_elems, key, kw, &pc, ar);
         if (vm.rdq() && kDiag == 0)
           rdq_push_lds(s, pc, round, rql);
         an.level(8, 0u);
@@ -647,7 +710,7 @@
   }
   int pc = -1;
   if (kDiag == 0 && lane < qn)
-    vote_row<R, M>(s, buf, round, qw[lane], st_rows, st_elems, key, &pc, ar);
+    vote_row<R, M>(s, buf, round, qw[lane], st_rows, st_elems, key, kw, &pc, ar);
   if (vm.rdq() && kDiag == 0)
     rdq_push_lds(s, pc, round, rql);
   if (an.on() && qn > 0)
@@ -758,7 +821,7 @@
   int nq = 0;
   if (lo < hi)
     nq = vote_waves<kBits, 8, kFilt, kDiag, M>(s, buf, round, lo, hi, bits, q + (threadIdx.x / kWave) * kQW, &st_rows,
-                                               &st_elems, s.key, &rql, an, ar);
+                                               &st_elems, s.key, key_win_ctl(s.ctl), &rql, an, ar);
   if (kRdq && kDiag == 0)
     rdq_flush_lds(s, round, &rql);
   if (an.on()) {
@@ -1250,7 +1313,8 @@
 }
 template <int K, int U>
 __device__ __forceinline__ int update_groups(const Dev& s, int64_t wbase, int64_t stride, int round, double prec,
-                                             bool* touch, int* ucnt_sh = nullptr, int32_t* ulist = nullptr,
+                                             bool* touch, const int32_t* kwc, int* ucnt_sh = nullptr,
+                                             int32_t* ulist = nullptr,
                                              Anat an = Anat(), UpdQuadLds<K>* ql = nullptr) {
   static_assert(upd_mode_ok(U), "not an update mode");
   constexpr bool kRdq = upd_mode(U).rdq(), kQuad = upd_mode(U).quad();
@@ -1449,7 +1513,7 @@
             rec->ratio = r;
           else
             wq = r;
-          const unsigned nk = ratio_key(r);
+          const unsigned nk = ratio_key(r, kwc ? key_win_ctl(kwc) : kKeyWinLegacy);
           s.key[c] = uint16_t(nk);
           changed = nk != okey[k];
           alive++;
@@ -1517,7 +1581,7 @@
   const int64_t stride = int64_t(gridDim.x) * kBlock;
   for (int64_t base = (int64_t(blockIdx.x) * kBlock + threadIdx.x) & ~int64_t(kWave - 1); base < s.nC;
        base += LMM_UPD_K * stride)
-    alive += update_groups<LMM_UPD_K, U>(s, base, stride, round, prec, &any_touch, &ucnt_sh, ulist, an, ql);
+    alive += update_groups<LMM_UPD_K, U>(s, base, stride, round, prec, &any_touch, s.ctl, &ucnt_sh, ulist, an, ql);
   const unsigned long long t_loop = an.now();
   if (alive)
     atomicAdd(&alive_cnt, alive);
@@ -1542,6 +1606,25 @@
       an.put(4 + f, an.lv(f));
     an.put(7, an.cnt(0));
     an.put(8, an.cnt(1));
+  }
+}
+
+__global__ void __launch_bounds__(kBlock) mm_key_diag(Dev s, int round) {
+  if (s.ctl[CTL_DONE])
+    return;
+  int n = 0, nt = 0;
+  for (int64_t c = int64_t(blockIdx.x) * kBlock + threadIdx.x; c < s.nC; c += int64_t(gridDim.x) * kBlock) {
+    const unsigned k = s.key[c];
+    const bool st = !key_dead(k) && s.chg[c] == uint16_t(round);
+    n += st;
+    nt += st && k == kKeyTop;
+  }
+  n = grp_isum<kWave>(n);
+  nt = grp_isum<kWave>(nt);
+  if ((threadIdx.x & (kWave - 1)) == 0 && n) {
+    atomicAdd(&s.ctl[CTL_KW_STORES], n);
+    if (nt)
+      atomicAdd(&s.ctl[CTL_KW_CLAMP], nt);
   }
 }
 
diff --git a/simgrid_amd/csrc/lmm_persist_kernels.hpp b/simgrid_amd/csrc/lmm_persist_kernels.hpp
--- a/simgrid_amd/csrc/lmm_persist_kernels.hpp
+++ b/simgrid_amd/csrc/lmm_persist_kernels.hpp
@@ -176,7 +176,8 @@
   int nq = 0;
   if (lo < hi)
     nq = vote_waves<kBits, R, kPFilt, 0, kVoteArrays>(s, buf, round, lo, hi, L.bits,
-                                                      L.q + (threadIdx.x / kWave) * kQW, &L.st0, &L.st1, s.key);
+                                                      L.q + (threadIdx.x / kWave) * kQW, &L.st0, &L.st1, s.key,
+                                                      kKeyWinLegacy);
   if (count) {
     if ((threadIdx.x & (kWave - 1)) == 0 && nq)
       atomicAdd(&L.st0, nq);
@@ -292,7 +293,10 @@
   if (!bar_rdv(b, rdv_ticks, hflag))
     return;
   unsigned gen = 0;
-  init_cnsts_waves(s, nullptr, prec, pwave(), int64_t(gridDim.x) * kPW);
+  {
+    double rlo = dinf(), rhi = 0.0;
+    init_cnsts_waves(s, nullptr, prec, pwave(), int64_t(gridDim.x) * kPW, rlo, rhi);
+  }
   init_vars_range<RowForm::Arrays>(s, int64_t(blockIdx.x) * kPB + threadIdx.x, int64_t(gridDim.x) * kPB);
   if (!grid_sync(b, ++gen))
     return;
@@ -319,7 +323,7 @@
       constexpr int kU = 3;
       const int64_t stride = int64_t(gridDim.x) * kPB;
       for (int64_t base = pwave() * kWave; base < s.nC; base += kU * stride)
-        alive += update_groups<kU, kUpdPlain>(s, base, stride, r, prec, &touch);
+        alive += update_groups<kU, kUpdPlain>(s, base, stride, r, prec, &touch, nullptr);
       alive = grp_isum<kWave>(alive);
       if (lane == 0 && alive)
         atomicAdd(&L.cnt, alive);
diff --git a/simgrid_amd/csrc/lmm_round_mode.hpp b/simgrid_amd/csrc/lmm_round_mode.hpp
--- a/simgrid_amd/csrc/lmm_round_mode.hpp
+++ b/simgrid_amd/csrc/lmm_round_mode.hpp
@@ -18,6 +18,7 @@
   constexpr bool rdq() const { return queue; }
   constexpr bool sat_retire() const { return filter; }
   constexpr bool tie_loads() const { return rec(); }
+  constexpr bool bound_keys() const { return rec(); }
   constexpr bool valid() const { return rec() || (!queue && !filter); }
   constexpr int index() const { return !rec() ? 0 : 1 + 4 * int(rec16()) + 2 * int(queue) + int(filter); }
 };
diff --git a/simgrid_amd/lmm.py b/simgrid_amd/lmm.py
--- a/simgrid_amd/lmm.py
+++ b/simgrid_amd/lmm.py
@@ -171,6 +171,7 @@
     "lmmhip_ctx_use_own_stream": (I, [P]),
     "lmmhip_ctx_set_engine": (I, [P, I]),
     "lmmhip_engine_fallbacks": (I, [P, PI64]),
+    "lmmhip_key_window": (I, [P, PI64]),
     "lmmhip_last_engine": (I, [P, PI]),
     "lmmhip_persist_profile": (I, [P, I, PI64, I64, PI64]),
     "lmmhip_persist_profile_blocks": (I, [P, PI64, I64, PI64, PI64]),
@@ -519,6 +520,11 @@
         _check_hip(lib().lmmhip_engine_fallbacks(self.device_ctx(), ct.byref(n)))
         return n.value
 
+    def key_window(self):
+        out = (ct.c_int64 * 4)()
+        _check_hip(lib().lmmhip_key_window(self.device_ctx(), out))
+        return dict(base=out[0], shift=out[1], key_stores=out[2], key_clamped=out[3])
+
     RAN_PERSISTENT, RAN_ROUNDS, RAN_FRONTIER, RAN_BATCH, RAN_FB_ROUNDS, RAN_FB_BATCH = range(6)
 
     def last_engine(self):
```

New measurement: 471.3 million (median of 6 runs). +1.4%, better.
